# Prachet-Dev-Singh/DenseCLIP_Vit_multimodal

Measured on AMD Instinct MI355X. Metric: images/sec (fwd+bwd) ViT-B/16 DenseCLIP @1024x2048, higher is better.
Workload: dtype bf16

## Files before the change

denseclip_vit_multimodal_amd/_native.py:

```python
import ctypes
import os
import threading

_HERE = os.path.dirname(os.path.abspath(__file__))
LIB_PATH = os.environ.get("DCLIP_LIB", os.path.join(_HERE, "libdclip.so"))

F32, F16, BF16 = 0, 1, 2
EPI_STORE, EPI_GELU, EPI_RESIDUAL, EPI_GELU_BWD, EPI_SPLITK, EPI_STORE_SCALED = 0, 1, 2, 3, 4, 5
OPT_ATTN_FWD_WAVES, OPT_ATTN_DQ_WAVES, OPT_ATTN_DKDV_WAVES, OPT_GEMM_TILE, OPT_GEMM_TN_TILE = 0, 1, 2, 3, 4
OPT_ATTN_DKDV_QS, OPT_ATTN_FWD_KERNEL, OPT_ATTN_BWD_KERNEL, OPT_ATTN_BWD_BLOCK, OPT_GEMM_TN_COLSUM = 5, 6, 7, 8, 9
OPT_GEMM_EPI, OPT_GEMM_TAIL, OPT_ATTN_FP8_QK, OPT_ATTN_DQ_ISSUE, OPT_ATTN_DQ_ROWS = 10, 11, 12, 13, 14
OPT_ATTN_DQ_DEFER, OPT_GEMM_SCHED, OPT_GEMM_KLOOP = 15, 16, 17
OPT_ATTN_DQ_REDUCE = 18
OPT_ATTN_PREP_ORDER = 19
OPT_ATTN_BWD_WGS = 20
OPT_ATTN_DQ_DEFER = 15

_c_void_p = ctypes.c_void_p
_i32 = ctypes.c_int
_i64 = ctypes.c_int64
_f32 = ctypes.c_float

_SIGS = {
    "dclip_layernorm_fwd": [_c_void_p, _i32, _c_void_p, _c_void_p, _c_void_p, _i32, _c_void_p, _c_void_p,
                            _i64, _i64, _f32, _c_void_p],
    "dclip_layernorm_bwd": [_c_void_p, _i32, _c_void_p, _i32, _c_void_p, _c_void_p, _c_void_p, _c_void_p, _i32,
                            _c_void_p, _c_void_p, _i64, _i64, _c_void_p],
    "dclip_layernorm_bwd_res": [_c_void_p, _i32, _c_void_p, _i64, _c_void_p, _i32, _c_void_p, _c_void_p, _c_void_p,
                                _c_void_p, _c_void_p, _c_void_p, _i32, _c_void_p, _c_void_p, _c_void_p, _i64, _i64,
                                _c_void_p],
    "dclip_layernorm_bwd_ws_floats": [_i64, _i64],
    "dclip_layernorm_bwd_add": [_c_void_p, _i32, _c_void_p, _c_void_p, _c_void_p, _c_void_p, _c_void_p, _c_void_p,
                                _i32, _c_void_p, _c_void_p, _i32, _c_void_p, _c_void_p, _c_void_p, _i64, _i64,
                                _c_void_p],
    "dclip_layernorm_bwd_scaled_add": [_c_void_p, _i32, _c_void_p, _c_void_p, _c_void_p, _c_void_p, _c_void_p,
                                       _c_void_p, _c_void_p, _i32, _c_void_p, _i32, _c_void_p, _c_void_p, _c_void_p,
                                       _c_void_p, _c_void_p, _i64, _i64, _f32, _c_void_p, _i32, _c_void_p, _c_void_p],
    "dclip_gemm": [_i32, _i32, _c_void_p, _i64, _c_void_p, _i64, _i64, _i64, _i64, _i32, _f32, _c_void_p, _c_void_p,
                   _c_void_p,
                   _i32, _i64, _c_void_p, _i32, _i64, _c_void_p, _i64, _c_void_p],
    "dclip_gemm_tn": [_i32, _i32, _c_void_p, _i64, _c_void_p, _i64, _i64, _i64, _i64, _i64, _i32, _f32, _c_void_p,
                      _c_void_p,
                      _c_void_p, _c_void_p, _i64, _c_void_p, _c_void_p],
    "dclip_attn_fwd": [_i32, _c_void_p, _c_void_p, _c_void_p, _i32, _i32, _i32, _i32, _f32, _c_void_p],
    "dclip_attn_bwd": [_i32, _c_void_p, _c_void_p, _c_void_p, _c_void_p, _c_void_p, _c_void_p, _i32, _i32, _i32,
                       _i32, _f32, _c_void_p],
    "dclip_im2col": [_c_void_p, _i32, _c_void_p, _i32, _i64, _i32, _i32, _i32, _i32, _i32, _c_void_p],
    "dclip_tokens_fwd": [_c_void_p, _i32, _c_void_p, _c_void_p, _c_void_p, _i32, _i32, _i32, _c_void_p],
    "dclip_tokens_bwd": [_c_void_p, _c_void_p, _i32, _f32, _c_void_p, _c_void_p, _c_void_p, _i32, _i32, _i32,
                         _c_void_p],
    "dclip_pos_interp_fwd": [_c_void_p, _c_void_p, _i32, _i32, _i32, _i32, _c_void_p],
    "dclip_pos_interp_bwd": [_c_void_p, _c_void_p, _i32, _i32, _i32, _i32, _c_void_p],
    "dclip_transpose": [_c_void_p, _i32, _i64, _i64, _i64, _c_void_p, _i32, _i64, _i64, _i32, _i64, _i64, _i64,
                        _i32, _c_void_p, _c_void_p],
    "dclip_weight_refresh": [_c_void_p, _i32, _i64, _i32, _c_void_p],
    "dclip_row_mean_workspace": [_i32, _i64, _i32],
    "dclip_row_mean": [_c_void_p, _i32, _i64, _i64, _i64, _i32, _i64, _i32, _c_void_p, _c_void_p, _c_void_p],
    "dclip_score_map": [_c_void_p, _i32, _i64, _i64, _i64, _c_void_p, _c_void_p, _i32, _i32, _i32, _i32, _f32,
                        _c_void_p],
    "dclip_score_concat": [_c_void_p, _i32, _i64, _i64, _i64, _i32, _c_void_p, _i32, _i32, _i32, _c_void_p, _i32, _i32,
                           _i32, _c_void_p],
    "dclip_bilinear_fwd": [_c_void_p, _i32, _c_void_p, _i32, _i64, _i32, _i32, _i32, _i32, _c_void_p],
    "dclip_bilinear_bwd": [_c_void_p, _i32, _c_void_p, _c_void_p, _i64, _i32, _i32, _i32, _i32, _c_void_p],
    "dclip_cast": [_c_void_p, _i32, _c_void_p, _i32, _i64, _f32, _c_void_p, _c_void_p],
    "dclip_grad_scale": [_c_void_p, _i64, _f32, _c_void_p, _c_void_p],
    "dclip_cityscapes_augment": [_c_void_p, _c_void_p, _c_void_p, _i32, _i32, _i32, _c_void_p, _i32, _i32,
                                 _c_void_p, _c_void_p, _f32, _f32, _c_void_p, _i32, _c_void_p, _c_void_p, _c_void_p,
                                 _c_void_p],
    "dclip_color_jitter": [_c_void_p, _i32, _i32, _i32, _c_void_p, _c_void_p, _c_void_p],
    "dclip_normalize_u8": [_c_void_p, _i32, _i32, _i32, _c_void_p, _c_void_p, _c_void_p, _i32, _c_void_p],
    "dclip_bn_eval": [_i32, _c_void_p, _i64, _i32, _i64, _c_void_p, _c_void_p, _f32, _c_void_p, _c_void_p,
                      _c_void_p, _c_void_p, _i32, _c_void_p],
    "dclip_row_scale_add": [_c_void_p, _c_void_p, _c_void_p, _i32, _c_void_p, _i64, _i32, _c_void_p],
    "dclip_add_readout_amax": [_c_void_p, _c_void_p, _i32, _c_void_p, _c_void_p, _i64, _i32, _i32, _f32, _c_void_p,
                               _c_void_p],
    "dclip_add_readout_cast": [_c_void_p, _c_void_p, _i32, _c_void_p, _c_void_p, _i32, _i64, _i32, _i32, _f32,
                               _c_void_p],
    "dclip_add_readout_cast_scaled": [_c_void_p, _c_void_p, _i32, _c_void_p, _c_void_p, _c_void_p, _i64, _i32, _i32,
                                      _f32, _c_void_p, _i32, _c_void_p, _c_void_p],
    "dclip_layernorm_bwd_scaled": [_c_void_p, _i32, _c_void_p, _c_void_p, _i32, _c_void_p, _c_void_p, _c_void_p,
                                   _c_void_p, _c_void_p, _c_void_p, _c_void_p, _c_void_p, _c_void_p, _i64, _i64, _f32,
                                   _c_void_p, _i32, _c_void_p, _c_void_p],
    "dclip_bn_workspace": [_i64, _i32],
    "dclip_bn_fwd": [_i32, _c_void_p, _i64, _i32, _i64, _c_void_p, _c_void_p, _f32, _f32, _c_void_p, _c_void_p,
                     _c_void_p, _c_void_p, _c_void_p, _c_void_p, _i32, _c_void_p],
    "dclip_bn_bwd": [_i32, _c_void_p, _c_void_p, _i64, _i32, _i64, _c_void_p, _c_void_p, _c_void_p, _c_void_p,
                     _c_void_p, _c_void_p, _c_void_p, _c_void_p, _i32, _c_void_p, _c_void_p],
    "dclip_conv3x3": [_i32, _i32, _c_void_p, _i64, _i64, _i64, _i32, _i32, _i32, _i32, _c_void_p, _i32, _c_void_p,
                      _i32, _i64, _i32, _i32, _i32, _c_void_p],
    "dclip_upsample_ce": [_i32, _c_void_p, _i32, _i32, _i32, _i32, _c_void_p, _i32, _i32, _i32, _i32, _c_void_p,
                          _c_void_p, _c_void_p, _c_void_p, _c_void_p],
    "dclip_upsample_silog": [_i32, _i32, _c_void_p, _i32, _i32, _i32, _c_void_p, _c_void_p, _i32, _i32, _f32, _f32,
                             _c_void_p, _c_void_p, _c_void_p, _c_void_p],
    "dclip_upsample_ws_floats": [_i32, _i32, _i32, _i32],
    "dclip_upsample_eval_ws_bytes": [_i32, _i32, _i32, _i32],
    "dclip_upsample_eval_seg": [_i32, _c_void_p, _i32, _i32, _i32, _i32, _c_void_p, _i32, _i32, _i32, _i32,
                                _c_void_p, _c_void_p, _c_void_p, _c_void_p, _c_void_p, _c_void_p],
    "dclip_upsample_eval_depth": [_i32, _c_void_p, _i32, _i32, _i32, _c_void_p, _c_void_p, _i32, _i32, _f32, _f32,
                                  _i32, _f32, _c_void_p, _c_void_p, _c_void_p, _c_void_p],
    "dclip_score_map_classes": [_c_void_p, _i32, _i64, _i64, _i64, _c_void_p, _c_void_p, _i32, _i32, _i32, _i32,
                                _f32, _c_void_p],
    "dclip_upsample_ce_classes_ws_floats": [_i32, _i32, _i32, _i32],
    "dclip_upsample_ce_classes": [_i32, _c_void_p, _i32, _i32, _i32, _i32, _c_void_p, _i32, _i32, _i32, _i32,
                                  _c_void_p, _c_void_p, _c_void_p, _c_void_p, _c_void_p],
    "dclip_upsample_ce_opt_ws_floats": [_i32, _i32, _i32, _i32],
    "dclip_upsample_ce_opt": [_i32, _c_void_p, _i32, _i32, _i32, _i32, _c_void_p, _i32, _i32, _i32, _i32,
                              _c_void_p, _f32, _c_void_p, _c_void_p, _c_void_p, _c_void_p, _c_void_p, _c_void_p,
                              _c_void_p],
    "dclip_upsample_eval_seg_classes_ws_bytes": [_i32, _i32, _i32, _i32],
    "dclip_upsample_eval_seg_classes": [_i32, _c_void_p, _i32, _i32, _i32, _i32, _c_void_p, _i32, _i32, _i32, _i32,
                                        _c_void_p, _c_void_p, _c_void_p, _c_void_p, _c_void_p, _c_void_p],
    "dclip_ensemble_eval_ws_bytes": [_i32, _i32, _i32],
    "dclip_ensemble_eval_seg": [_i32, _c_void_p, _i32, _i32, _i32, _i32, _c_void_p, _i32, _i32, _i32, _i32,
                                _c_void_p, _c_void_p, _c_void_p, _c_void_p, _c_void_p, _c_void_p],
    "dclip_ensemble_eval_depth": [_i32, _c_void_p, _i32, _i32, _c_void_p, _c_void_p, _i32, _i32, _f32, _f32,
                                  _i32, _f32, _c_void_p, _c_void_p, _c_void_p, _c_void_p],
    "dclip_slide_eval_ws_bytes": [_i32, _i32, _i32],
    "dclip_slide_eval_seg": [_i32, _c_void_p, _i32, _i32, _i32, _i32, _i32, _i32, _i32, _c_void_p, _i32, _i32, _i32,
                             _i32, _c_void_p, _c_void_p, _c_void_p, _c_void_p, _c_void_p, _c_void_p],
    "dclip_slide_eval_depth": [_i32, _c_void_p, _i32, _i32, _i32, _i32, _i32, _i32, _c_void_p, _c_void_p, _i32, _i32,
                               _f32, _f32, _i32, _f32, _c_void_p, _c_void_p, _c_void_p, _c_void_p],
    "dclip_slide_tta_eval_ws_bytes": [_i32, _i32, _i32, _i32],
    "dclip_slide_tta_eval_seg": [_i32, _c_void_p, _i32, _c_void_p, _i32, _i32, _i32, _i32, _c_void_p, _i32, _i32,
                                 _i32, _i32, _c_void_p, _c_void_p, _c_void_p, _c_void_p, _c_void_p, _c_void_p],
    "dclip_slide_tta_eval_depth": [_i32, _c_void_p, _i32, _c_void_p, _i32, _i32, _c_void_p, _c_void_p, _i32, _i32,
                                   _f32, _f32, _i32, _f32, _c_void_p, _c_void_p, _c_void_p, _c_void_p],
    "dclip_conv3x3_wgrad": [_i32, _c_void_p, _i64, _i32, _c_void_p, _i64, _i64, _i64, _i32, _i32, _i32, _i32,
                            _c_void_p, _c_void_p, _i32, _i32, _c_void_p, _c_void_p],
    "dclip_set_option": [_i32, _i32],
    "dclip_cityscapes_prepare": [_c_void_p, _c_void_p, _c_void_p, _i32, _i32, _i32, _c_void_p, _i32, _i32,
                                 _c_void_p, _c_void_p, _f32, _f32, _c_void_p, _i32, _c_void_p, _c_void_p, _c_void_p,
                                 _c_void_p],
    "dclip_attn_bwd_workspace": [_i32, _i32, _i32],
    "dclip_attn_bwd_fp8_workspace": [_i32, _i32, _i32],
    "dclip_attn_bwd_fp8": [_i32, _c_void_p, _c_void_p, _c_void_p, _c_void_p, _c_void_p, _c_void_p, _i32, _i32, _i32,
                           _i32, _f32, _c_void_p],
    "dclip_attn_fwd_fp8": [_i32, _c_void_p, _c_void_p, _c_void_p, _c_void_p, _i32, _i32, _i32, _i32, _c_void_p],
    "dclip_attn_fwd_fp8_workspace": [_i32, _i32, _i32],
    "dclip_gemm_tn_plan": [_i64, _i64, _i64, _c_void_p, _c_void_p],
    "dclip_adamw_ws_bytes": [_i64],
    "dclip_adamw_prepare": [_c_void_p, _c_void_p, _c_void_p, _i32, _i64, _c_void_p, _i32, _c_void_p, _c_void_p,
                            _c_void_p, _i32, _c_void_p],
    "dclip_adamw_update": [_c_void_p, _c_void_p, _c_void_p, _i32, _i64, _c_void_p, _c_void_p],
}
EXPORTED = sorted(list(_SIGS) + ["dclip_last_error", "dclip_abi_version"])
ENSEMBLE_MAX_VIEWS = 16
CLASSES_MAX = 256


class View(ctypes.Structure):
    _fields_ = [("low", ctypes.c_void_p), ("h", ctypes.c_int), ("w", ctypes.c_int), ("flip", ctypes.c_int)]


def view_table(views):
    return (View * len(views))(*[View(p, int(h), int(w), int(f)) for p, h, w, f in views])


SLIDE_MAX_WINDOWS = 64


class Window(ctypes.Structure):
    _fields_ = [("low", ctypes.c_void_p), ("y0", ctypes.c_int), ("x0", ctypes.c_int)]


def window_table(windows):
    return (Window * len(windows))(*[Window(p, int(y), int(x)) for p, y, x in windows])


SLIDE_TTA_MAX_WINDOWS = 1024


class SlideView(ctypes.Structure):
    _fields_ = [(n, ctypes.c_int) for n in ("Hv", "Wv", "flip", "wh", "ww", "h", "w", "first", "nwin")]


def slide_view_table(views):
    return (SlideView * len(views))(*[SlideView(*[int(c) for c in v]) for v in views])


_lib = None
_lock = threading.Lock()


class NativeError(RuntimeError):
    pass


def load(path=None):
    global _lib
    with _lock:
        if _lib is not None and path is None:
            return _lib
        p = path or LIB_PATH
        if not os.path.exists(p):
            raise NativeError(
                f"libdclip.so not found at {p}: build it with `make -C denseclip_vit_multimodal_amd/csrc` "
                "(the HIP path has no CPU fallback)")
        lib = ctypes.CDLL(p)
        for name, args in _SIGS.items():
            fn = getattr(lib, name)
            fn.argtypes = args
            fn.restype = ctypes.c_int
        lib.dclip_last_error.restype = ctypes.c_char_p
        lib.dclip_last_error.argtypes = []
        lib.dclip_abi_version.restype = ctypes.c_int
        lib.dclip_abi_version.argtypes = []
        lib.dclip_attn_bwd_workspace.restype = ctypes.c_int64
        lib.dclip_attn_bwd_fp8_workspace.restype = ctypes.c_int64
        lib.dclip_bn_workspace.restype = ctypes.c_int64
        lib.dclip_attn_fwd_fp8_workspace.restype = ctypes.c_int64
        lib.dclip_row_mean_workspace.restype = ctypes.c_int64
        lib.dclip_layernorm_bwd_ws_floats.restype = ctypes.c_int64
        lib.dclip_upsample_ws_floats.restype = ctypes.c_int64
        lib.dclip_upsample_eval_ws_bytes.restype = ctypes.c_int64
        lib.dclip_upsample_ce_classes_ws_floats.restype = ctypes.c_int64
        lib.dclip_upsample_ce_opt_ws_floats.restype = ctypes.c_int64
        lib.dclip_upsample_eval_seg_classes_ws_bytes.restype = ctypes.c_int64
        lib.dclip_adamw_ws_bytes.restype = ctypes.c_int64
        lib.dclip_ensemble_eval_ws_bytes.restype = ctypes.c_int64
        lib.dclip_slide_eval_ws_bytes.restype = ctypes.c_int64
        lib.dclip_slide_tta_eval_ws_bytes.restype = ctypes.c_int64
        for kv in filter(None, os.environ.get("DCLIP_OPTIONS", "").split(",")):
            k, v = kv.split("=")
            if lib.dclip_set_option(int(k), int(v)) != 0:
                raise NativeError(f"DCLIP_OPTIONS: {lib.dclip_last_error().decode()}")
        if path is None:
            _lib = lib
        return lib


def lib():
    return load()


def call(name, *args):
    L = load()
    rc = getattr(L, name)(*args)
    if rc != 0:
        msg = L.dclip_last_error().decode(errors="replace")
        raise NativeError(f"{name} failed ({rc}): {msg}")
    return rc
```

denseclip_vit_multimodal_amd/_torch_ops.py:

```python
import os

import torch

_HERE = os.path.dirname(os.path.abspath(__file__))
LIB_PATH = os.environ.get("DCLIP_TORCH_LIB", os.path.join(_HERE, "libdclip_torch.so"))

_loaded = False


def load():
    global _loaded
    if _loaded:
        return torch.ops.dclip
    if not os.path.exists(LIB_PATH):
        raise RuntimeError(f"libdclip_torch.so not found at {LIB_PATH}: build it with "
                           "`make -C denseclip_vit_multimodal_amd/csrc` (the HIP path has no CPU fallback)")
    from . import _native
    bound = os.path.realpath(os.path.join(os.path.dirname(LIB_PATH), "libdclip.so"))
    if os.path.realpath(_native.LIB_PATH) != bound:
        raise RuntimeError(f"DCLIP_LIB ({_native.LIB_PATH}) is not the libdclip.so that {LIB_PATH} binds ({bound}); "
                           "build a matching adapter and point DCLIP_TORCH_LIB at it")
    _native.load()
    torch.ops.load_library(LIB_PATH)
    _register_fakes()
# ... 211 lines not shown
    @reg("dclip_eval::seg_update")
    def _(logits, labels, ignore_index, cm, ce_sums, want_pred):
        return _e(*labels.shape, like=logits, dtype=torch.uint8) if want_pred else None

    @reg("dclip_eval::depth_update")
    def _(pred, target, mask, min_depth, max_depth, clamp_pred, eps, sums, want_up):
        B, H, W = target.shape
        return _e(B, 1, H, W, like=pred, dtype=f32) if want_up else None

    @reg("dclip_eval::ensemble_argmax")
    def _(logits, flips, H, W, probs):
        return _e(logits[0].shape[0], H, W, like=logits[0], dtype=torch.uint8)

    @reg("dclip_eval::ensemble_seg_update")
    def _(logits, flips, labels, ignore_index, probs, cm, ce_sums, want_pred):
        return _e(*labels.shape, like=logits[0], dtype=torch.uint8) if want_pred else None

    @reg("dclip_eval::ensemble_depth")
    def _(preds, flips, H, W):
        return _e(preds[0].shape[0], 1, H, W, like=preds[0], dtype=f32)

    @reg("dclip_eval::ensemble_depth_update")
    def _(preds, flips, target, mask, min_depth, max_depth, clamp_pred, eps, sums, want_up):
        B, H, W = target.shape
        return _e(B, 1, H, W, like=preds[0], dtype=f32) if want_up else None

    @reg("dclip_eval::slide_argmax")
    def _(logits, origins, wh, ww, H, W):
        return _e(logits[0].shape[0], H, W, like=logits[0], dtype=torch.uint8)

    @reg("dclip_eval::slide_seg_update")
    def _(logits, origins, wh, ww, labels, ignore_index, cm, ce_sums, want_pred):
        return _e(*labels.shape, like=logits[0], dtype=torch.uint8) if want_pred else None

    @reg("dclip_eval::slide_depth")
    def _(preds, origins, wh, ww, H, W):
        return _e(preds[0].shape[0], 1, H, W, like=preds[0], dtype=f32)

    @reg("dclip_eval::slide_depth_update")
    def _(preds, origins, wh, ww, target, mask, min_depth, max_depth, clamp_pred, eps, sums, want_up):
        B, H, W = target.shape
        return _e(B, 1, H, W, like=preds[0], dtype=f32) if want_up else None

    @reg("dclip_eval::slide_tta_argmax")
    def _(logits, views, origins, H, W, probs):
        return _e(logits[0].shape[0], H, W, like=logits[0], dtype=torch.uint8)

    @reg("dclip_eval::slide_tta_seg_update")
    def _(logits, views, origins, labels, ignore_index, probs, cm, ce_sums, want_pred):
        return _e(*labels.shape, like=logits[0], dtype=torch.uint8) if want_pred else None

    @reg("dclip_eval::slide_tta_depth")
    def _(preds, views, origins, H, W):
        return _e(preds[0].shape[0], 1, H, W, like=preds[0], dtype=f32)

    @reg("dclip_eval::slide_tta_depth_update")
    def _(preds, views, origins, target, mask, min_depth, max_depth, clamp_pred, eps, sums, want_up):
        B, H, W = target.shape
        return _e(B, 1, H, W, like=preds[0], dtype=f32) if want_up else None

    @reg("dclip_eval::upsample_argmax_classes")
    def _(logits, H, W):
        return _e(logits.shape[0], H, W, like=logits, dtype=torch.uint8)

    @reg("dclip_eval::seg_update_classes")
    def _(logits, labels, ignore_index, cm, ce_sums, want_pred, ws=None):
        return _e(*labels.shape, like=logits, dtype=torch.uint8) if want_pred else None

    @reg("dclip_classes::score_map")
    def _(v, bstride, row_off, ld, text, B, HW, eps):
        return _e(B, text.shape[1], HW, like=v, dtype=f32)

    @reg("dclip_classes::upsample_ce")
    def _(logits, labels, ignore_index):
        return (_e(1, like=logits, dtype=torch.float64), _e(1, like=logits, dtype=torch.int32),
                _e(*logits.shape, like=logits, dtype=f32))

    @reg("dclip_loss::upsample_ce")
    def _(logits, labels, ignore_index, class_weight, label_smoothing, pixel_weight, want_pixel_loss, want_grad):
        return (_e(2, like=logits, dtype=torch.float64), _e(1, like=logits, dtype=torch.int32),
                _e(*logits.shape, like=logits, dtype=f32) if want_grad else None,
                _e(*labels.shape, like=logits, dtype=f32) if want_pixel_loss else None)

    @reg("dclip_optim::adamw_prepare")
    def _(desc, desc_host, grads, tiles, hp, found_inf, state, with_norm):
        return None

    @reg("dclip_optim::adamw_update")
    def _(desc, desc_host, grads, tiles, state):
        return None
```

denseclip_vit_multimodal_amd/csrc/gemm.hip:

```cpp
#include <mutex>
#include <type_traits>

#include "common.h"

namespace {

constexpr int BM = 128, BN = 128, BK = 64;
constexpr int TILE_BYTES = 128 * BK * 2;
constexpr int STAGE_BYTES = 2 * TILE_BYTES;
constexpr int EP_LD = 68;
constexpr int SMEM_BYTES = 4 * 64 * EP_LD * 4 > 2 * STAGE_BYTES ? 4 * 64 * EP_LD * 4 : 2 * STAGE_BYTES;

template <typename T>
__device__ __forceinline__ void store8(T* p, const float* v, bool full, int rem) {
    if (full) {
        if constexpr (sizeof(T) == 4) {
            f32x4 a = {v[0], v[1], v[2], v[3]}, b = {v[4], v[5], v[6], v[7]};
            *(f32x4*)p = a;
            *(f32x4*)(p + 4) = b;
        } else {
            typedef T t8 __attribute__((ext_vector_type(8)));
            t8 x;
#pragma unroll
            for (int e = 0; e < 8; ++e) x[e] = (T)v[e];
// ... 719 lines not shown
            for (int q = 0; q < 4; ++q) {
                const int rr = (lane >> 4) + 4 * q, cc = lane & 15;
                f32x4 x = *(const f32x4*)(img + rr * 256 + ((cc ^ (rr & 15)) * 16));
                const int64_t row = row0 + rr;
                const int col = nw + 4 * cc;
                if constexpr (EPI == DCLIP_EPI_RESIDUAL) {
                    x += cur[q];
                    st16<NTS>((f32x4*)((float*)C + row * ldc + col), x);
                    if (C2 != nullptr) {
                        const t4 y = {(T)x[0], (T)x[1], (T)x[2], (T)x[3]};
                        *(t4*)((T*)C2 + row * ldc2 + col) = y;
                    }
                } else if constexpr (EPI == DCLIP_EPI_GELU_BWD) {
#pragma unroll
                    for (int e = 0; e < 4; ++e) x[e] *= quick_gelu_grad((float)cur[q][e]);
                    store4_out<OutT>((OutT*)C + row * ldc + col, x);
                } else {
                    store4_out<OutT>((OutT*)C + row * ldc + col, x);
                }
            }
        } else {
#pragma unroll
            for (int q = 0; q < 2; ++q) {
                const int rr = (lane >> 3) + 8 * q, cc = lane & 7;
                const int off = rr * 128 + ((cc ^ ((rr >> 1) & 7)) * 16);
                const int64_t row = row0 + rr;
                const int col = nw + 8 * cc;
                if (EPI != DCLIP_EPI_GELU || C != nullptr)
                    st16<NTS>((u32x4*)((OutT*)C + row * ldc + col), *(const u32x4*)(img + off));
                if constexpr (EPI == DCLIP_EPI_GELU)
                    st16<NTS>((u32x4*)((OutT*)C2 + row * ldc2 + col), *(const u32x4*)(img + 2048 + off));
            }
        }
        asm volatile("" ::: "memory");
        if constexpr (AUX) {
            if (j + 1 < Cfg::MB) {
#pragma unroll
                for (int q = 0; q < 4; ++q) cur[q] = nxt[q];
            }
        }
    }
}

__device__ __forceinline__ void pers_range(int x, int G, int ntiles, int& lo, int& hi) {
    const int rest = ntiles - G;
    lo = G + (int)((int64_t)rest * x / 8);
    hi = G + (int)((int64_t)rest * (x + 1) / 8);
}

__device__ __forceinline__ int pers_resolve(unsigned* __restrict__ sched, int v, int xcd, int G, int ntiles) {
    int lo, hi;
    pers_range(xcd, G, ntiles, lo, hi);
    if (lo + v < hi) return lo + v;
#pragma unroll 1
    for (int k = 1; k < 8; ++k) {
        const int x = (xcd + k) & 7;
        pers_range(x, G, ntiles, lo, hi);
        if (lo >= hi) continue;
        const int w = (int)atomicAdd(sched + 32 * x, 1u);
        if (lo + w < hi) return lo + w;
    }
    unsigned* const bm = sched + 288;
#pragma unroll 1
    for (int w = 0; w < (G + 31) / 32; ++w) {
        const unsigned valid = (w * 32 + 32 <= G) ? 0xffffffffu : ((1u << (G - w * 32)) - 1u);
        unsigned bits = atomicOr(bm + w, 0u);
        while ((~bits & valid) != 0u) {
            const int bit = __builtin_ctz(~bits & valid);
            const unsigned old = atomicOr(bm + w, 1u << bit);
            if (!(old & (1u << bit))) return w * 32 + bit;
            bits |= old;
        }
    }
    if ((int)atomicAdd(sched + 256, 1u) == G - 1) {
#pragma unroll 1
        for (int i = 0; i < 8; ++i) atomicExch(sched + 32 * i, 0u);
        atomicExch(sched + 256, 0u);
#pragma unroll 1
        for (int i = 288; i < 296; ++i) atomicExch(sched + i, 0u);
    }
    return ntiles;
}

template <typename T, int EPI, typename OutT, int NW = 8, bool ELDS = false, bool DYN = false, bool NTS = false,
          bool PF = false>
__global__ __launch_bounds__(64 * NW, 1) void gemm_nt_pers_kernel(
    const T* __restrict__ A, int64_t lda, const T* __restrict__ B, int64_t ldb, int K, int tiles_m, int tiles_n,
    const float* __restrict__ bias, const void* __restrict__ aux, int64_t ld_aux, void* __restrict__ C, int64_t ldc,
    void* __restrict__ C2, int64_t ldc2, Alpha alpha_arg, unsigned* __restrict__ sched = nullptr) {
    const float alpha = alpha_arg.get();
    typedef BigCfg<256, 256, 2, NW / 2, 2, 64> Cfg;
    typedef typename Mfma<T>::frag frag;
    constexpr int EPI_IMG = (NW == 8 && ELDS) ? 4096 : 0;
    __shared__ __attribute__((aligned(16))) char smem[Cfg::SMEM + NW * EPI_IMG];
    const int lane = threadIdx.x & 63;
    const int wave = __builtin_amdgcn_readfirstlane(threadIdx.x >> 6);
    const int wm = wave / (NW / 2), wn = wave % (NW / 2);
    constexpr bool epi_lds = NW == 8 && ELDS;
    const int l16 = lane & 15, lq = lane >> 4;
    const int ntiles = tiles_m * tiles_n;
    const int G = gridDim.x;
    const int r = xcd_remap(blockIdx.x, G);
    const int nk = K / 64;
    const int M = tiles_m * 256, N = tiles_n * 256;

    const uint32_t abytes = (uint32_t)((int64_t)M * lda * sizeof(T)), bbytes = (uint32_t)((int64_t)N * ldb * sizeof(T));
    const uint32_t lda_b = (uint32_t)(lda * sizeof(T)), ldb_b = (uint32_t)(ldb * sizeof(T));
    uint32_t va[2], vb[2];
    rows_voff2<Cfg::A_INST>(lda_b, lane, va);
    rows_voff2<Cfg::B_INST>(ldb_b, lane, vb);
#define PERS_STAGE(M0, N0, KT, SLOT)                                                                                 \
    do {                                                                                                             \
        char* base_ = smem + (SLOT) * Cfg::STAGE_BYTES;                                                              \
        const uint32_t kb_ = (uint32_t)((KT) * 64 * sizeof(T));                                                      \
        stage_rows_sbuf<T, Cfg::A_INST>(A, abytes, va, (uint32_t)((M0) + 8 * wave * Cfg::A_INST) * lda_b + kb_,     \
                                        8 * lda_b, base_, wave);                                                     \
        stage_rows_sbuf<T, Cfg::B_INST>(B, bbytes, vb, (uint32_t)((N0) + 8 * wave * Cfg::B_INST) * ldb_b + kb_,     \
                                        8 * ldb_b, base_ + Cfg::A_BYTES, wave);                                      \
    } while (0)
    int u = r;
    if (u >= ntiles) return;
    int m0 = (u / tiles_n) * 256, n0 = (u % tiles_n) * 256;
    int* const pub = (int*)(smem + Cfg::SMEM);
    const int xcd = blockIdx.x & 7;
    unsigned own_old = 0;
    int pend = 0;
    if constexpr (DYN) {
        static_assert(!DYN || (NW == 8 && ELDS), "the claim words live in wave 0's epilogue image");
        if (threadIdx.x == 0) {
            own_old = atomicOr(sched + 288 + (r >> 5), 1u << (r & 31));
            pend = (int)atomicAdd(sched + 32 * xcd, 1u);
        }
    }
    PERS_STAGE(m0, n0, 0, 0);
    int slot = 0;
    bool first = true;
    while (true) {
        f32x4 acc[Cfg::NB][Cfg::MB];
#pragma unroll
        for (int i = 0; i < Cfg::NB; ++i)
#pragma unroll
            for (int j = 0; j < Cfg::MB; ++j) acc[i][j] = f32x4{0.f, 0.f, 0.f, 0.f};
        PersCols<EPI, Cfg::NB> pc;
        pers_cols<EPI, Cfg::NB>(pc, bias, aux, n0 + wn * Cfg::WTN, lq);
        int un = u + G;
        if constexpr (DYN) {
            if (nk == 2 && threadIdx.x == 0) {
                pub[0] = pers_resolve(sched, pend, xcd, G, ntiles);
                asm volatile("s_waitcnt lgkmcnt(0)" ::: "memory");
            }
        }
        int nm0 = (un / tiles_n) * 256, nn0 = (un % tiles_n) * 256;
        bool skip = false;
        for (int kt = 0; kt < nk; ++kt) {
            if (kt == 0 && !first) wait_vmcnt<PERS_EPI_MIN>();
            else wait_vmcnt<0>();
            if constexpr (DYN) {
                if (kt == 0 && first && u == r && threadIdx.x == 0) {
                    pub[1] = (own_old >> (r & 31)) & 1u;
                    asm volatile("s_waitcnt lgkmcnt(0)" ::: "memory");
                }
            }
            __builtin_amdgcn_s_barrier();
            __builtin_amdgcn_sched_barrier(0);
            if constexpr (DYN) {
                if (kt == 0 && first && u == r && __builtin_amdgcn_readfirstlane(pub[1]) != 0) {
                    skip = true;
                    break;
                }
                if (kt == nk - 2) {
                    un = __builtin_amdgcn_readfirstlane(pub[0]);
                    nm0 = (un / tiles_n) * 256;
                    nn0 = (un % tiles_n) * 256;
                }
            }
            if (kt + 1 < nk) {
                PERS_STAGE(m0, n0, kt + 1, slot ^ 1);
            } else if (un < ntiles) {
                PERS_STAGE(nm0, nn0, 0, slot ^ 1);
            }
            const char* At = smem + slot * Cfg::STAGE_BYTES;
            const char* Bt = At + Cfg::A_BYTES;
            if constexpr (PF && NW == 8) {
                frag fb[2][Cfg::NB], fa[4];
                auto rd_b = [&](int ks) {
#pragma unroll
                    for (int i = 0; i < Cfg::NB; ++i)
// ... 885 lines not shown
            __syncthreads();
        }
    }
    if constexpr (AD) __syncthreads();
    gemm_epilogue<T, DCLIP_EPI_SPLITK, float>(acc, smem, M, N, m0, n0, nullptr, nullptr, 0, C, N, nullptr, 0, slab,
                                               1.0f);
}

const void* conv_zero_row() {
    static void* z = nullptr;
    if (!z) {
        if (hipMalloc(&z, 256) != hipSuccess) return nullptr;
        if (hipMemset(z, 0, 256) != hipSuccess) return nullptr;
    }
    return z;
}

float* tail_scratch(size_t floats) {
    static float* buf = nullptr;
    static size_t cap = 0;
    if (floats > cap) {
        if (buf) (void)hipFree(buf);
        buf = nullptr;
        cap = 0;
        if (hipMalloc(&buf, floats * sizeof(float)) != hipSuccess) return nullptr;
        cap = floats;
    }
    return buf;
}

template <typename T, int EPI, typename OutT>
__global__ __launch_bounds__(512) void gemm_tail16_kernel(const T* __restrict__ A, int64_t lda, const T* __restrict__ B,
                                                          int64_t ldb, int mt, int N, int K, int m0,
                                                          const float* __restrict__ bias, const void* __restrict__ aux,
                                                          int64_t ld_aux, void* __restrict__ C, int64_t ldc,
                                                          void* __restrict__ C2, int64_t ldc2, Alpha alpha_arg) {
    typedef typename Mfma<T>::frag frag;
    __shared__ float red[8][16][68];
    const int lane = threadIdx.x & 63, wave = threadIdx.x >> 6;
    const int l16 = lane & 15, lq = lane >> 4;
    const int n0 = blockIdx.x * 64;
    const int ks = K / 8, kbeg = wave * ks;
    const bool rowok = l16 < mt;
    const T* arow = A + (int64_t)(rowok ? l16 : 0) * lda + kbeg + 8 * lq;
    const T* brow = B + (int64_t)(n0 + l16) * ldb + kbeg + 8 * lq;
    f32x4 acc[4];
#pragma unroll
    for (int i = 0; i < 4; ++i) acc[i] = f32x4{0.f, 0.f, 0.f, 0.f};
    frag zf;
#pragma unroll
    for (int j = 0; j < 8; ++j) zf[j] = (T)0.f;
#pragma unroll 4
    for (int k = 0; k < ks; k += 32) {
        const frag a = rowok ? *(const frag*)(arow + k) : zf;
        frag b[4];
#pragma unroll
        for (int i = 0; i < 4; ++i) b[i] = *(const frag*)(brow + (int64_t)16 * i * ldb + k);
#pragma unroll
        for (int i = 0; i < 4; ++i) acc[i] = Mfma16<T>::mma(a, b[i], acc[i]);
    }
#pragma unroll
    for (int i = 0; i < 4; ++i)
#pragma unroll
        for (int e = 0; e < 4; ++e) red[wave][4 * lq + e][16 * i + l16] = acc[i][e];
    __syncthreads();
    const int t = threadIdx.x;
    if (t < 128) {
        const int r = t >> 3, cb = (t & 7) * 8;
        if (r < mt) {
            const float alpha = alpha_arg.get();
            float v[8];
#pragma unroll
            for (int e = 0; e < 8; ++e) {
                float sum = 0.f;
#pragma unroll
                for (int w = 0; w < 8; ++w) sum += red[w][r][cb + e];
                v[e] = sum * alpha;
            }
            epi_row8<T, EPI, OutT>(v, m0 + r, n0 + cb, N, bias, aux, ld_aux, C, ldc, C2, ldc2, 0);
        }
    }
}

template <typename T, int EPI, typename OutT>
__global__ __launch_bounds__(1024) void gemm_tail16x16_kernel(const T* __restrict__ A, int64_t lda,
                                                              const T* __restrict__ B, int64_t ldb, int mt, int N,
                                                              int W, int IT, int m0, const float* __restrict__ bias,
                                                              const void* __restrict__ aux, int64_t ld_aux,
                                                              void* __restrict__ C, int64_t ldc, void* __restrict__ C2,
                                                              int64_t ldc2, Alpha alpha_arg) {
    typedef typename Mfma<T>::frag frag;
    constexpr int ITMAX = 6;
    __shared__ float red[16][16][17];
    const int lane = threadIdx.x & 63, wave = threadIdx.x >> 6;
    const int l16 = lane & 15, lq = lane >> 4;
    const int n0 = blockIdx.x * 16;
    const int t = threadIdx.x;
    const int er = t >> 1, ecb = (t & 1) * 8;
    const bool epi = t < 2 * mt;
    float bv[8], pre[8];
#pragma unroll
    for (int e = 0; e < 8; ++e) bv[e] = pre[e] = 0.f;
    if (epi) {
        const int nb = n0 + ecb;
        if (bias != nullptr && EPI != DCLIP_EPI_GELU_BWD) load8<float>(bias + nb, bv, true, 8);
        if constexpr (EPI == DCLIP_EPI_STORE_SCALED) load8<float>((const float*)aux + nb, pre, true, 8);
        if constexpr (EPI == DCLIP_EPI_RESIDUAL)
            load8<float>((const float*)aux + (int64_t)(m0 + er) * ld_aux + nb, pre, true, 8);
        if constexpr (EPI == DCLIP_EPI_GELU_BWD) load8<T>((const T*)aux + (int64_t)(m0 + er) * ld_aux + nb, pre, true, 8);
    }
    const bool rowok = l16 < mt;
    const int kbeg = wave * IT * 32;
    const T* arow = A + (int64_t)(rowok ? l16 : 0) * lda + kbeg + 8 * lq;
    const T* brow = B + (int64_t)(n0 + l16) * ldb + kbeg + 8 * lq;
    frag zf;
#pragma unroll
    for (int j = 0; j < 8; ++j) zf[j] = (T)0.f;
    frag a[ITMAX], b[ITMAX];
#pragma unroll
    for (int it = 0; it < ITMAX; ++it) {
        if (it < IT) {
            a[it] = rowok ? *(const frag*)(arow + 32 * it) : zf;
            b[it] = *(const frag*)(brow + 32 * it);
        }
    }
    f32x4 acc = f32x4{0.f, 0.f, 0.f, 0.f};
#pragma unroll
    for (int it = 0; it < ITMAX; ++it)
        if (it < IT) acc = Mfma16<T>::mma(a[it], b[it], acc);
#pragma unroll
    for (int e = 0; e < 4; ++e) red[wave][4 * lq + e][l16] = acc[e];
    __syncthreads();
    if (epi) {
        const float alpha = alpha_arg.get();
        float v[8];
#pragma unroll
        for (int e = 0; e < 8; ++e) {
            float sum = 0.f;
            for (int w = 0; w < W; ++w) sum += red[w][er][ecb + e];
            v[e] = sum * alpha + bv[e];
        }
        const int64_t m = m0 + er;
        const int nb = n0 + ecb;
        if constexpr (EPI == DCLIP_EPI_STORE) {
            store8<OutT>((OutT*)C + m * ldc + nb, v, true, 8);
        } else if constexpr (EPI == DCLIP_EPI_STORE_SCALED) {
#pragma unroll
            for (int e = 0; e < 8; ++e) v[e] *= pre[e];
            store8<OutT>((OutT*)C + m * ldc + nb, v, true, 8);
        } else if constexpr (EPI == DCLIP_EPI_GELU) {
            float g[8];
#pragma unroll
            for (int e = 0; e < 8; ++e) {
                v[e] = (float)(OutT)v[e];
                g[e] = quick_gelu(v[e]);
            }
            if (C != nullptr) store8<OutT>((OutT*)C + m * ldc + nb, v, true, 8);
            store8<OutT>((OutT*)C2 + m * ldc2 + nb, g, true, 8);
        } else if constexpr (EPI == DCLIP_EPI_RESIDUAL) {
#pragma unroll
            for (int e = 0; e < 8; ++e) v[e] += pre[e];
            store8<float>((float*)C + m * ldc + nb, v, true, 8);
            if (C2 != nullptr) store8<T>((T*)C2 + m * ldc2 + nb, v, true, 8);
        } else if constexpr (EPI == DCLIP_EPI_GELU_BWD) {
#pragma unroll
            for (int e = 0; e < 8; ++e) v[e] *= quick_gelu_grad(pre[e]);
            store8<OutT>((OutT*)C + m * ldc + nb, v, true, 8);
        }
    }
}

inline bool tail16x16_plan(int64_t K, int& W, int& IT) {
    if (K % 32 != 0) return false;
    const int s = (int)(K / 32);
    for (int w = 16; w >= 1; --w)
        if (s % w == 0 && s / w <= 6) {
            W = w;
            IT = s / w;
            return true;
        }
    return false;
}

template <typename T, int EPI, typename OutT>
__global__ void tail_combine_kernel(const float* __restrict__ ws, int splits, int rows, int N, int64_t m0,
                                    const float* __restrict__ bias, const void* __restrict__ aux, int64_t ld_aux,
                                    void* __restrict__ C, int64_t ldc, void* __restrict__ C2, int64_t ldc2) {
    const int n8 = (N + 7) / 8;
    const int i = blockIdx.x * blockDim.x + threadIdx.x;
    if (i >= rows * n8) return;
    const int r = i / n8, nb = (i % n8) * 8;
    const bool full = nb + 8 <= N;
    float v[8] = {0.f, 0.f, 0.f, 0.f, 0.f, 0.f, 0.f, 0.f};
    for (int sp = 0; sp < splits; ++sp) {
        float t[8];
        load8<float>(ws + ((int64_t)sp * rows + r) * N + nb, t, full, N - nb);
#pragma unroll
        for (int e = 0; e < 8; ++e) v[e] += t[e];
    }
    epi_row8<T, EPI, OutT>(v, (int)(m0 + r), nb, N, bias, aux, ld_aux, C, ldc, C2, ldc2, 0);
}

template <typename T, int EPI, typename OutT, int TBM, int TBN, int WM, int WN, int STAGES, int BKT = 64,
          bool PP = false>
void launch_big(const void* A, int64_t lda, const void* B, int64_t ldb, int64_t M, int64_t N, int64_t K,
                int splits, Alpha alpha, const float* bias, const void* aux, int64_t ld_aux, void* C, int64_t ldc,
                void* C2, int64_t ldc2, hipStream_t st) {
    int tiles_m = (int)((M + TBM - 1) / TBM);
    const int tiles_n = (int)((N + TBN - 1) / TBN);
    const int64_t Mfull = (M / TBM) * TBM, tail = M - Mfull;
    auto rounds = [](int64_t t) { return (t + 255) / 256; };
    if (EPI != DCLIP_EPI_SPLITK && splits == 1 && tail > 0 && tail <= 64 && Mfull > 0 && K >= 1536 &&
        rounds((int64_t)tiles_m * tiles_n) > rounds((Mfull / TBM) * tiles_n)) {
        const int ksteps = (int)(K / BKT);
        int ts = 1;
        for (int c = 16; c >= 1; --c)
            if (ksteps % c == 0) {
                ts = c;
                break;
            }
        float* ws = tail_scratch((size_t)ts * tail * N);
        if (ws != nullptr) {
            tiles_m = (int)(Mfull / TBM);
            const int ttm = 1;
            gemm_nt_big_kernel<T, DCLIP_EPI_SPLITK, float, TBM, TBN, WM, WN, STAGES, BKT>
                <<<dim3(ttm * tiles_n, ts), 64 * WM * WN, 0, st>>>(
                    (const T*)A + Mfull * lda, lda, (const T*)B, ldb, (int)tail, (int)N, (int)(K / ts), ttm, tiles_n,
                    nullptr, nullptr, 0, ws, N, nullptr, 0, tail * N, alpha);
            const int threads = (int)(tail * ((N + 7) / 8));
            tail_combine_kernel<T, EPI, OutT><<<(threads + 255) / 256, 256, 0, st>>>(
                ws, ts, (int)tail, (int)N, Mfull, bias, aux, ld_aux, C, ldc, C2, ldc2);
            M = Mfull;
        }
    }
    dim3 grid(tiles_m * tiles_n, splits);
    if constexpr (PP) {
        static_assert(TBM == 256 && TBN == 256 && WM == 2 && WN == 4, "ping-pong geometry");
        gemm_nt_pp_kernel<T, EPI, OutT><<<grid, 512, 0, st>>>(
            (const T*)A, lda, (const T*)B, ldb, (int)M, (int)N, (int)(K / splits), tiles_m, tiles_n, bias, aux, ld_aux,
            C, ldc, C2, ldc2, (int64_t)M * N, alpha);
    } else {
        gemm_nt_big_kernel<T, EPI, OutT, TBM, TBN, WM, WN, STAGES, BKT><<<grid, 64 * WM * WN, 0, st>>>(
            (const T*)A, lda, (const T*)B, ldb, (int)M, (int)N, (int)(K / splits), tiles_m, tiles_n, bias, aux,
            ld_aux, C, ldc, C2, ldc2, (int64_t)M * N, alpha);
    }
}

int cu_count() {
    static int n[64] = {0};
    int dev = 0;
    (void)hipGetDevice(&dev);
    if (dev < 0 || dev >= 64) return 256;
    if (n[dev] == 0) {
        int c = 0;
        if (hipDeviceGetAttribute(&c, hipDeviceAttributeMultiprocessorCount, dev) != hipSuccess || c <= 0) c = 256;
        n[dev] = c;
    }
    return n[dev];
}

unsigned* gemm_sched_counters(hipStream_t st) {
    static std::mutex mu;
    static unsigned* base[64] = {nullptr};
    static hipStream_t owner[64][64];
    static int used[64] = {0};
    if (dclip_option(DCLIP_OPT_GEMM_SCHED) != 1) return nullptr;
    hipStreamCaptureStatus cs = hipStreamCaptureStatusNone;
    if (hipStreamIsCapturing(st, &cs) != hipSuccess || cs != hipStreamCaptureStatusNone) return nullptr;
    int dev = 0;
    if (hipGetDevice(&dev) != hipSuccess || dev < 0 || dev >= 64) return nullptr;
    std::lock_guard<std::mutex> lock(mu);
    if (base[dev] == nullptr) {
        unsigned* p = nullptr;
        const size_t bytes = 64 * 512 * sizeof(unsigned);
        if (hipMalloc(&p, bytes) != hipSuccess) return nullptr;
        if (hipMemset(p, 0, bytes) != hipSuccess) {
            (void)hipFree(p);
            return nullptr;
        }
        base[dev] = p;
    }
    for (int i = 0; i < used[dev]; ++i)
        if (owner[dev][i] == st) return base[dev] + 512 * i;
    if (used[dev] == 64) return nullptr;
    owner[dev][used[dev]] = st;
    return base[dev] + 512 * used[dev]++;
}

inline bool pers_streaming_stores(int epi, int64_t N) {
    const int o = dclip_option(DCLIP_OPT_GEMM_EPI);
    if (o == 2) return true;
    if (o != 0) return false;
    return N >= 2048 && epi != DCLIP_EPI_GELU_BWD && epi != DCLIP_EPI_RESIDUAL;
}

inline bool pers_prefetch_kloop(int epi) {
    const int o = dclip_option(DCLIP_OPT_GEMM_KLOOP);
    if (o == 1) return true;
    if (o != 0) return false;
    return epi != DCLIP_EPI_GELU;
}

template <typename T, int EPI, typename OutT, int NW = 8, bool PIPE = false>
bool launch_pers(const void* A, int64_t lda, const void* B, int64_t ldb, int64_t M, int64_t N, int64_t K,
                 Alpha alpha, const float* bias, const void* aux, int64_t ld_aux, void* C, int64_t ldc, void* C2,
                 int64_t ldc2, hipStream_t st) {
    if constexpr (EPI == DCLIP_EPI_SPLITK) {
        return false;
    } else {
        const int64_t Mfull = (M / 256) * 256, tail = M - Mfull;
        const int G = cu_count();
        if (N % 256 != 0 || tail > 64 || (Mfull / 256) * (N / 256) < 2 * G) return false;
        if (PIPE && K < 128) return false;
        if (Mfull * lda * (int64_t)sizeof(T) >= (1ll << 32) || N * ldb * (int64_t)sizeof(T) >= (1ll << 32)) return false;
        if (EPI == DCLIP_EPI_STORE_SCALED || (bias != nullptr && EPI != DCLIP_EPI_GELU_BWD)) {
            if (((uintptr_t)(EPI == DCLIP_EPI_STORE_SCALED ? aux : bias) % 16) != 0) return false;
            if (bias != nullptr && ((uintptr_t)bias % 16) != 0) return false;
        }
        if (ldc % 4 != 0 || (C2 != nullptr && ldc2 % 4 != 0) || (EPI == DCLIP_EPI_RESIDUAL && ld_aux % 4 != 0) ||
            (EPI == DCLIP_EPI_GELU_BWD && ld_aux % 4 != 0))
            return false;
        const int tail_opt = dclip_option(DCLIP_OPT_GEMM_TAIL);
        int tw = 0, tit = 0;
        if (tail > 0 && tail <= 16 && tail_opt == 0 && tail16x16_plan(K, tw, tit)) {
            gemm_tail16x16_kernel<T, EPI, OutT><<<(unsigned)(N / 16), 64 * tw, 0, st>>>(
                (const T*)A + Mfull * lda, lda, (const T*)B, ldb, (int)tail, (int)N, tw, tit, (int)Mfull, bias, aux,
                ld_aux, C, ldc, C2, ldc2, alpha);
        } else if (tail > 0 && tail <= 16 && K % 256 == 0 && tail_opt != 1) {
            gemm_tail16_kernel<T, EPI, OutT><<<(unsigned)(N / 64), 512, 0, st>>>(
                (const T*)A + Mfull * lda, lda, (const T*)B, ldb, (int)tail, (int)N, (int)K, (int)Mfull, bias, aux,
                ld_aux, C, ldc, C2, ldc2, alpha);
        } else if (tail > 0) {
            const int tiles_n = (int)(N / 256);
            const int ksteps = (int)(K / 64);
            int ts = 1;
            for (int c = 16; c >= 1; --c)
                if (ksteps % c == 0) {
                    ts = c;
                    break;
                }
            float* ws = tail_scratch((size_t)ts * tail * N);
            if (ws == nullptr) return false;
            gemm_nt_big_kernel<T, DCLIP_EPI_SPLITK, float, 256, 256, 2, 4, 2, 64>
                <<<dim3(tiles_n, ts), 512, 0, st>>>((const T*)A + Mfull * lda, lda, (const T*)B, ldb, (int)tail, (int)N,
                                                    (int)(K / ts), 1, tiles_n, nullptr, nullptr, 0, ws, N, nullptr, 0,
                                                    tail * N, alpha);
            const int threads = (int)(tail * ((N + 7) / 8));
            tail_combine_kernel<T, EPI, OutT><<<(threads + 255) / 256, 256, 0, st>>>(
                ws, ts, (int)tail, (int)N, Mfull, bias, aux, ld_aux, C, ldc, C2, ldc2);
        }
        if constexpr (PIPE)
            gemm_nt_pipe_kernel<T, EPI, OutT, NW><<<G, 64 * NW, 0, st>>>((const T*)A, lda, (const T*)B, ldb, (int)K,
                                                                         (int)(Mfull / 256), (int)(N / 256), bias, aux,
                                                                         ld_aux, C, ldc, C2, ldc2, alpha);
        else
        {
            unsigned* sched = (NW == 8 && dclip_option(DCLIP_OPT_GEMM_EPI) != 1 && K >= 128 && G <= 256)
                                  ? gemm_sched_counters(st)
                                  : nullptr;
            if (sched != nullptr)
                gemm_nt_pers_kernel<T, EPI, OutT, NW, true, NW == 8><<<G, 64 * NW, 0, st>>>(
                    (const T*)A, lda, (const T*)B, ldb, (int)K, (int)(Mfull / 256), (int)(N / 256), bias, aux, ld_aux, C,
                    ldc, C2, ldc2, alpha, sched);
#define PERS_LAUNCH(NTS_, PF_)                                                                                  \
    gemm_nt_pers_kernel<T, EPI, OutT, NW, true, false, NTS_, PF_><<<G, 64 * NW, 0, st>>>(                        \
        (const T*)A, lda, (const T*)B, ldb, (int)K, (int)(Mfull / 256), (int)(N / 256), bias, aux, ld_aux, C, ldc, C2, \
        ldc2, alpha)
            else if (NW == 8 && dclip_option(DCLIP_OPT_GEMM_EPI) != 1) {
                const bool nts = pers_streaming_stores(EPI, N), pf = pers_prefetch_kloop(EPI);
                if (nts && pf) PERS_LAUNCH(true, true);
                else if (nts) PERS_LAUNCH(true, false);
                else if (pf) PERS_LAUNCH(false, true);
                else PERS_LAUNCH(false, false);
            }
#undef PERS_LAUNCH
            else
                gemm_nt_pers_kernel<T, EPI, OutT, NW, false><<<G, 64 * NW, 0, st>>>(
                    (const T*)A, lda, (const T*)B, ldb, (int)K, (int)(Mfull / 256), (int)(N / 256), bias, aux, ld_aux, C,
                    ldc, C2, ldc2, alpha);
        }
        return true;
    }
}

inline int gemm_tile_choice(int64_t M, int64_t N) {
    const int opt = dclip_option(DCLIP_OPT_GEMM_TILE);
    if (opt != 0) return opt;
    if (M < 4096) return 1;
    return 6;
}

template <typename T, int EPI, typename OutT>
int launch(const void* A, int64_t lda, const void* B, int64_t ldb, int64_t M, int64_t N, int64_t K,
           int splits, Alpha alpha, const float* bias, const void* aux, int64_t ld_aux, void* C, int64_t ldc,
           void* C2, int64_t ldc2, hipStream_t st) {
    const int choice = gemm_tile_choice(M, N);
    if (choice == 2) {
        launch_big<T, EPI, OutT, 256, 256, 2, 4, 2>(A, lda, B, ldb, M, N, K, splits, alpha, bias, aux, ld_aux, C,
                                                    ldc, C2, ldc2, st);
        return 0;
    }
    if (choice == 3) {
        launch_big<T, EPI, OutT, 256, 128, 4, 2, 3>(A, lda, B, ldb, M, N, K, splits, alpha, bias, aux, ld_aux, C,
                                                    ldc, C2, ldc2, st);
        return 0;
    }
    if (choice == 6 && splits == 1 &&
        launch_pers<T, EPI, OutT>(A, lda, B, ldb, M, N, K, alpha, bias, aux, ld_aux, C, ldc, C2, ldc2, st))
        return 0;
    if (choice == 7 && splits == 1 &&
        launch_pers<T, EPI, OutT, 4>(A, lda, B, ldb, M, N, K, alpha, bias, aux, ld_aux, C, ldc, C2, ldc2, st))
        return 0;
    if (choice == 8 && splits == 1 &&
        launch_pers<T, EPI, OutT, 8, true>(A, lda, B, ldb, M, N, K, alpha, bias, aux, ld_aux, C, ldc, C2, ldc2, st))
        return 0;
    if (choice == 9 && splits == 1 &&
        launch_pers<T, EPI, OutT, 4, true>(A, lda, B, ldb, M, N, K, alpha, bias, aux, ld_aux, C, ldc, C2, ldc2, st))
        return 0;
    if (choice >= 6) {
        launch_big<T, EPI, OutT, 256, 256, 2, 4, 2>(A, lda, B, ldb, M, N, K, splits, alpha, bias, aux, ld_aux, C,
                                                    ldc, C2, ldc2, st);
        return 0;
    }
    if (choice == 5) {
        launch_big<T, EPI, OutT, 256, 256, 2, 4, 2, 64, true>(A, lda, B, ldb, M, N, K, splits, alpha, bias, aux,
                                                              ld_aux, C, ldc, C2, ldc2, st);
        return 0;
    }
    if (choice == 4) {
        launch_big<T, EPI, OutT, 256, 256, 2, 4, 4, 32>(A, lda, B, ldb, M, N, K, splits, alpha, bias, aux, ld_aux, C,
                                                        ldc, C2, ldc2, st);
        return 0;
    }
    const int tiles_m = (int)((M + BM - 1) / BM), tiles_n = (int)((N + BN - 1) / BN);
    const int k_chunk = (int)(K / splits);
    dim3 grid(tiles_m * tiles_n, splits);
    gemm_nt_kernel<T, EPI, OutT><<<grid, 256, 0, st>>>(
        (const T*)A, lda, (const T*)B, ldb, (int)M, (int)N, k_chunk, tiles_m, tiles_n, bias, aux,
        ld_aux, C, ldc, C2, ldc2, (int64_t)M * N, alpha);
    return 0;
}

template <typename T>
int dispatch(int epi, int c_dt, const void* A, int64_t lda, const void* B, int64_t ldb, int64_t M,
             int64_t N, int64_t K, int splits, Alpha alpha, const float* bias, const void* aux, int64_t ld_aux,
             void* C, int64_t ldc, void* C2, int64_t ldc2, hipStream_t st) {
    switch (epi) {
        case DCLIP_EPI_STORE:
            if (c_dt == DCLIP_F32)
                return launch<T, DCLIP_EPI_STORE, float>(A, lda, B, ldb, M, N, K, 1, alpha, bias, aux, ld_aux, C, ldc, C2, ldc2, st);
            return launch<T, DCLIP_EPI_STORE, T>(A, lda, B, ldb, M, N, K, 1, alpha, bias, aux, ld_aux, C, ldc, C2, ldc2, st);
        case DCLIP_EPI_STORE_SCALED:
            return launch<T, DCLIP_EPI_STORE_SCALED, T>(A, lda, B, ldb, M, N, K, 1, alpha, bias, aux, ld_aux, C, ldc, C2, ldc2, st);
        case DCLIP_EPI_GELU:
            return launch<T, DCLIP_EPI_GELU, T>(A, lda, B, ldb, M, N, K, 1, alpha, bias, aux, ld_aux, C, ldc, C2, ldc2, st);
        case DCLIP_EPI_RESIDUAL:
            return launch<T, DCLIP_EPI_RESIDUAL, float>(A, lda, B, ldb, M, N, K, 1, alpha, bias, aux, ld_aux, C, ldc, C2, ldc2, st);
        case DCLIP_EPI_GELU_BWD:
            return launch<T, DCLIP_EPI_GELU_BWD, T>(A, lda, B, ldb, M, N, K, 1, alpha, bias, aux, ld_aux, C, ldc, C2, ldc2, st);
        case DCLIP_EPI_SPLITK: {
            float* ws = (float*)const_cast<void*>(aux);
            launch<T, DCLIP_EPI_SPLITK, float>(A, lda, B, ldb, M, N, K, splits, alpha, nullptr, nullptr, 0,
// ... 275 lines not shown
```

denseclip_vit_multimodal_amd/csrc/misc.hip:

```cpp
#include "common.h"

namespace {

template <typename T>
__device__ __forceinline__ T cvt(float v) { return (T)v; }

template <typename TI, typename TO>
__global__ void im2col_kernel(const TI* __restrict__ img, TO* __restrict__ out, int B, int Cin, int Hin, int Win,
                              int p, int gh, int gw, int64_t ldo, int64_t total4) {
    const int64_t i = (int64_t)blockIdx.x * blockDim.x + threadIdx.x;
    if (i >= total4) return;
    const int64_t l4 = ldo / 4;
    const int64_t row = i / l4;
    const int col = (int)(i % l4) * 4;
    TO* dst = out + row * ldo + col;
    if (col >= Cin * p * p) {
#pragma unroll
        for (int e = 0; e < 4; ++e) dst[e] = (TO)0.0f;
        return;
    }
    const int kx = col % p, ky = (col / p) % p, cc = col / (p * p);
    const int px = (int)(row % gw);
    const int py = (int)((row / gw) % gh);
    const int b = (int)(row / ((int64_t)gw * gh));
// ... 894 lines not shown
    }
}

template <typename TB>
__global__ __launch_bounds__(256) void add_readout_cast_ds_kernel(const float* a, const TB* __restrict__ b,
                                                                  const float* __restrict__ bsc, float* sum,
                                                                  f16* __restrict__ lp, int64_t rows, int cols,
                                                                  int ntok, float target, float* __restrict__ st,
                                                                  int use, float* __restrict__ spair) {
    const int c8 = cols / 8;
    const int64_t n8 = rows * c8;
    const float sb = bsc != nullptr ? *bsc : 1.0f;
    const float ls = ds_scale_of_use(st, use, target);
    ds_begin(st, use, ls, spair);
    uint32_t m = 0;
    const int64_t stride = (int64_t)gridDim.x * blockDim.x;
    for (int64_t i = (int64_t)blockIdx.x * blockDim.x + threadIdx.x; i < n8; i += 2 * stride) {
        const int64_t i2 = i + stride;
        const bool two = i2 < n8;
        f32x4 x[4];
        readout_sum8<TB>(a, b, sb, i * 8, (i / c8) % ntok != 0, x[0], x[1]);
        if (two) readout_sum8<TB>(a, b, sb, i2 * 8, (i2 / c8) % ntok != 0, x[2], x[3]);
#pragma unroll
        for (int h = 0; h < 2; ++h) {
            if (h == 1 && !two) break;
            const int64_t off = (h ? i2 : i) * 8;
            if (b != nullptr) {
                *(f32x4*)(sum + off) = x[2 * h];
                *(f32x4*)(sum + off + 4) = x[2 * h + 1];
            }
            f16x8 o;
#pragma unroll
            for (int e = 0; e < 4; ++e) {
                m = max(m, max(__float_as_uint(x[2 * h][e]) & 0x7fffffffu, __float_as_uint(x[2 * h + 1][e]) & 0x7fffffffu));
                o[e] = (f16)(x[2 * h][e] * ls);
                o[4 + e] = (f16)(x[2 * h + 1][e] * ls);
            }
            *(f16x8*)(lp + off) = o;
        }
    }
    ds_end<4>(m, st, use);
}

extern "C" int dclip_add_readout_cast_scaled(const float* a, const void* b, int b_dt, const float* b_scale_ptr,
                                             float* sum, void* lp, int64_t rows, int cols, int ntok, float target,
                                             float* st, int use, float* spair, void* stream) {
    DCLIP_HOST_CHECK(cols % 8 == 0 && ntok > 0 && rows > 0 && target > 0.f && st != nullptr && spair != nullptr &&
                         use >= 1,
                     "dclip_add_readout_cast_scaled: cols %% 8 == 0, ntok > 0, rows > 0, target > 0, st, use >= 1, spair");
    DCLIP_HOST_CHECK(b == nullptr || sum != nullptr, "dclip_add_readout_cast_scaled: sum is required with b");
    DCLIP_HOST_CHECK(((uintptr_t)a | (uintptr_t)b | (uintptr_t)sum | (uintptr_t)lp) % 16 == 0,
                     "dclip_add_readout_cast_scaled: unaligned buffers");
    hipStream_t s = (hipStream_t)stream;
    const unsigned g = grid_for((rows * (cols / 8) + 1) / 2, 4096);
    if (b == nullptr) b_dt = DCLIP_F32;
    DISPATCH_DT(b_dt, TB,
        add_readout_cast_ds_kernel<TB><<<g, 256, 0, s>>>(a, (const TB*)b, b_scale_ptr, sum, (f16*)lp, rows, cols, ntok,
                                                         target, st, use, spair));
    DCLIP_LAUNCH_CHECK();
    return 0;
}

extern "C" int dclip_cast(const void* in, int in_dt, void* out, int out_dt, int64_t n, float scale_v,
                          const float* scale_ptr, void* stream) {
    if (n == 0) return 0;
    const Alpha scale(scale_v, scale_ptr);
    hipStream_t st = (hipStream_t)stream;
    DISPATCH_DT(in_dt, TI, DISPATCH_DT(out_dt, TO,
        cast_kernel<TI, TO><<<grid_for((n + 3) / 4), 256, 0, st>>>((const TI*)in, (TO*)out, n, scale)));
    DCLIP_LAUNCH_CHECK();
    return 0;
}

namespace {

constexpr int BN_NBLK_MAX = 512;

inline int bn_nblk(int64_t rows, int C) {
    const int rpb = 256 / (C / 8);
    const int64_t need = (rows + rpb - 1) / rpb;
    return (int)(need < BN_NBLK_MAX ? need : BN_NBLK_MAX);
}

template <typename T>
__device__ __forceinline__ void load8(const T* p, float* v) {
    typedef T t8 __attribute__((ext_vector_type(8)));
    const t8 r = *(const t8*)p;
#pragma unroll
    for (int e = 0; e < 8; ++e) v[e] = (float)r[e];
}

__device__ __forceinline__ void bn_affine8(const float* w, const float* b, const float* mean, const float* rstd, int c0,
                                           float* sc, float* sh) {
#pragma unroll
    for (int e = 0; e < 8; ++e) {
        sc[e] = (w ? w[c0 + e] : 1.f) * rstd[c0 + e];
        sh[e] = (b ? b[c0 + e] : 0.f) - mean[c0 + e] * sc[e];
    }
}

template <typename T, int MODE, bool RELU>
__global__ void __launch_bounds__(256) bn_stats_kernel(const T* __restrict__ a, const T* __restrict__ x,
                                                       const float* __restrict__ w, const float* __restrict__ b,
                                                       const float* __restrict__ mean, const float* __restrict__ rstd,
                                                       int64_t rows, int C, int64_t ld, float* __restrict__ part) {
    __shared__ float red[2 * 2048];
    const int tpr = C / 8, rpb = 256 / tpr;
    const int c8 = threadIdx.x % tpr, rr = threadIdx.x / tpr;
    float s[8], q[8], ref[8], sc[8], sh[8];
#pragma unroll
    for (int e = 0; e < 8; ++e) s[e] = q[e] = 0.f;
    if (rr < rpb) {
        if (MODE == 0) load8(a + c8 * 8, ref);
        else
#pragma unroll
            for (int e = 0; e < 8; ++e) ref[e] = mean[c8 * 8 + e];
        if (RELU) bn_affine8(w, b, mean, rstd, c8 * 8, sc, sh);
#pragma unroll 4
        for (int64_t r = (int64_t)blockIdx.x * rpb + rr; r < rows; r += (int64_t)gridDim.x * rpb) {
            float v[8];
            load8(a + r * ld + c8 * 8, v);
            if (MODE == 0) {
#pragma unroll
                for (int e = 0; e < 8; ++e) {
                    const float d = v[e] - ref[e];
                    s[e] += d;
                    q[e] += d * d;
                }
            } else {
                float xv[8];
                load8(x + r * ld + c8 * 8, xv);
#pragma unroll
                for (int e = 0; e < 8; ++e) {
                    const float g = (!RELU || xv[e] * sc[e] + sh[e] > 0.f) ? v[e] : 0.f;
                    s[e] += g;
                    q[e] += g * (xv[e] - ref[e]);
                }
            }
        }
#pragma unroll
        for (int e = 0; e < 8; ++e) {
            red[rr * C + c8 * 8 + e] = s[e];
            red[2048 + rr * C + c8 * 8 + e] = q[e];
        }
    }
    __syncthreads();
    for (int c = threadIdx.x; c < C; c += 256) {
        float ss = 0.f, qq = 0.f;
        for (int k = 0; k < rpb; ++k) {
            ss += red[k * C + c];
            qq += red[2048 + k * C + c];
        }
        part[(int64_t)blockIdx.x * 2 * C + c] = ss;
        part[(int64_t)blockIdx.x * 2 * C + C + c] = qq;
    }
}

__device__ __forceinline__ void bn_reduce_parts(const float* __restrict__ part, int nblk, int C, int& c, float& S,
                                                float& Q) {
    __shared__ float red[2][32][8];
    const int lc = threadIdx.x & 7, grp = threadIdx.x >> 3;
    c = blockIdx.x * 8 + lc;
    float s = 0.f, q = 0.f;
    if (c < C) {
#pragma unroll 4
        for (int k = grp; k < nblk; k += 32) {
            s += part[(int64_t)k * 2 * C + c];
            q += part[(int64_t)k * 2 * C + C + c];
        }
    }
    red[0][grp][lc] = s;
    red[1][grp][lc] = q;
    __syncthreads();
    S = Q = 0.f;
    if (threadIdx.x < 8)
        for (int g = 0; g < 32; ++g) {
            S += red[0][g][lc];
            Q += red[1][g][lc];
        }
}

template <typename T>
__global__ void bn_fwd_finalize_kernel(const float* __restrict__ part, int nblk, const T* __restrict__ x, int64_t rows,
                                       int C, const float* __restrict__ w, const float* __restrict__ b, float eps,
                                       float momentum, float* __restrict__ rmean, float* __restrict__ rvar,
                                       float* __restrict__ mean, float* __restrict__ rstd, float* __restrict__ ss) {
    int c;
    float S, Q;
    bn_reduce_parts(part, nblk, C, c, S, Q);
    if (threadIdx.x >= 8 || c >= C) return;
    const float n = (float)rows;
    const float md = S / n;
    const float var = fmaxf(Q / n - md * md, 0.f);
    const float mu = (float)x[c] + md;
    const float rs = rsqrtf(var + eps);
    mean[c] = mu;
    rstd[c] = rs;
    const float sc = (w ? w[c] : 1.f) * rs;
    ss[c] = sc;
    ss[C + c] = (b ? b[c] : 0.f) - mu * sc;
    if (rmean) {
        rmean[c] = (1.f - momentum) * rmean[c] + momentum * mu;
        rvar[c] = (1.f - momentum) * rvar[c] + momentum * var * (rows > 1 ? n / (n - 1.f) : 1.f);
    }
}

__global__ void bn_bwd_finalize_kernel(const float* __restrict__ part, int nblk, int64_t rows, int C,
                                       const float* __restrict__ w, const float* __restrict__ mean,
                                       const float* __restrict__ rstd, float* __restrict__ dw, float* __restrict__ db,
                                       float* __restrict__ k, const float* __restrict__ gscale) {
    int c;
    float S, Q;
    bn_reduce_parts(part, nblk, C, c, S, Q);
    if (threadIdx.x >= 8 || c >= C) return;
    const float n = (float)rows, rs = rstd[c], wc = w ? w[c] : 1.f;
    const float ga = gscale ? *gscale : 1.f;
    if (dw) dw[c] = Q * rs * ga;
    if (db) db[c] = S * ga;
    const float k1 = wc * rs;
    const float k2 = -wc * rs * rs * rs * (Q / n);
    k[c] = k1;
    k[C + c] = k2;
    k[2 * C + c] = -k1 * (S / n) - k2 * mean[c];
}

template <typename T, bool BWD, bool RELU>
__global__ void __launch_bounds__(256) bn_apply_kernel(const T* __restrict__ a, const T* __restrict__ x,
                                                       const float* __restrict__ k, int64_t rows, int C, int64_t ld,
                                                       T* __restrict__ y) {
    const int c8n = C / 8;
    const int64_t n8 = rows * c8n;
    typedef T t8 __attribute__((ext_vector_type(8)));
    for (int64_t i = (int64_t)blockIdx.x * blockDim.x + threadIdx.x; i < n8; i += (int64_t)gridDim.x * blockDim.x) {
        const int c0 = (int)(i % c8n) * 8;
        const int64_t off = (i / c8n) * ld + c0;
        float v[8];
        load8(a + off, v);
        t8 o;
        if (BWD) {
            float xv[8];
            load8(x + off, xv);
#pragma unroll
            for (int e = 0; e < 8; ++e) {
                const float g = (!RELU || xv[e] * k[3 * C + c0 + e] + k[4 * C + c0 + e] > 0.f) ? v[e] : 0.f;
                o[e] = (T)(g * k[c0 + e] + xv[e] * k[C + c0 + e] + k[2 * C + c0 + e]);
            }
        } else {
#pragma unroll
            for (int e = 0; e < 8; ++e) {
                const float t = v[e] * k[c0 + e] + k[C + c0 + e];
                o[e] = (T)(RELU ? fmaxf(t, 0.f) : t);
            }
        }
        *(t8*)(y + off) = o;
    }
}

__global__ void bn_mask_affine_kernel(const float* __restrict__ w, const float* __restrict__ b,
                                      const float* __restrict__ mean, const float* __restrict__ rstd, int C,
                                      float* __restrict__ k) {
    const int c = blockIdx.x * 256 + threadIdx.x;
    if (c >= C) return;
    const float sc = (w ? w[c] : 1.f) * rstd[c];
    k[3 * C + c] = sc;
    k[4 * C + c] = (b ? b[c] : 0.f) - mean[c] * sc;
}

__global__ void bn_eval_affine_kernel(const float* __restrict__ w, const float* __restrict__ b,
                                      const float* __restrict__ rmean, const float* __restrict__ rvar, float eps,
                                      int C, float* __restrict__ ss) {
    const int c = blockIdx.x * 256 + threadIdx.x;
    if (c >= C) return;
    const float sc = (w ? w[c] : 1.f) / sqrtf(rvar[c] + eps);
    ss[c] = sc;
    ss[C + c] = (b ? b[c] : 0.f) - rmean[c] * sc;
}

bool bn_shape_ok(int64_t rows, int C, int64_t ld) {
    const int tpr = C / 8;
    return rows > 0 && C % 8 == 0 && tpr >= 1 && tpr <= 256 && ld >= C && ld % 8 == 0;
}

}

extern "C" int64_t dclip_bn_workspace(int64_t rows, int C) {
    (void)rows;
    return (int64_t)BN_NBLK_MAX * 2 * C + 5 * (int64_t)C;
}

extern "C" int dclip_bn_fwd(int dt, const void* x, int64_t rows, int C, int64_t ld, const float* w, const float* b,
                            float eps, float momentum, float* running_mean, float* running_var, float* ws, float* mean,
                            float* rstd, void* y, int relu, void* stream) {
    DCLIP_HOST_CHECK(dt == DCLIP_BF16 || dt == DCLIP_F16, "dclip_bn_fwd: dtype must be bf16/f16");
    DCLIP_HOST_CHECK(bn_shape_ok(rows, C, ld), "dclip_bn_fwd: need rows > 0, C %% 8 == 0, C <= 2048, ld >= C, "
                     "ld %% 8 == 0 (C = %d)", C);
    DCLIP_HOST_CHECK(((uintptr_t)x % 16) == 0 && ((uintptr_t)y % 16) == 0, "dclip_bn_fwd: unaligned buffers");
    hipStream_t st = (hipStream_t)stream;
    const int nblk = bn_nblk(rows, C);
    float* ss = ws + (int64_t)BN_NBLK_MAX * 2 * C;
    const unsigned ga = grid_for(rows * (C / 8), 8192);
#define BN_FWD(T)                                                                                                      \
    bn_stats_kernel<T, 0, false><<<nblk, 256, 0, st>>>((const T*)x, nullptr, nullptr, nullptr, nullptr, nullptr, rows, \
                                                       C, ld, ws);                                                     \
    bn_fwd_finalize_kernel<T><<<(C + 7) / 8, 256, 0, st>>>(ws, nblk, (const T*)x, rows, C, w, b, eps, momentum,        \
                                                           running_mean, running_var, mean, rstd, ss);                 \
    if (relu) bn_apply_kernel<T, false, true><<<ga, 256, 0, st>>>((const T*)x, nullptr, ss, rows, C, ld, (T*)y);       \
    else bn_apply_kernel<T, false, false><<<ga, 256, 0, st>>>((const T*)x, nullptr, ss, rows, C, ld, (T*)y);
    if (dt == DCLIP_BF16) {
        BN_FWD(bf16)
    } else {
        BN_FWD(f16)
    }
#undef BN_FWD
    DCLIP_LAUNCH_CHECK();
    return 0;
}

extern "C" int dclip_bn_eval(int dt, const void* x, int64_t rows, int C, int64_t ld, const float* w, const float* b,
                             float eps, const float* running_mean, const float* running_var, float* ws, void* y,
                             int relu, void* stream) {
    DCLIP_HOST_CHECK(dt == DCLIP_BF16 || dt == DCLIP_F16, "dclip_bn_eval: dtype must be bf16/f16");
    DCLIP_HOST_CHECK(bn_shape_ok(rows, C, ld), "dclip_bn_eval: need rows > 0, C %% 8 == 0, C <= 2048, ld >= C, "
                     "ld %% 8 == 0 (C = %d)", C);
    DCLIP_HOST_CHECK(running_mean && running_var && ws, "dclip_bn_eval: running statistics and workspace required");
    DCLIP_HOST_CHECK(((uintptr_t)x % 16) == 0 && ((uintptr_t)y % 16) == 0, "dclip_bn_eval: unaligned buffers");
    hipStream_t st = (hipStream_t)stream;
    float* ss = ws + (int64_t)BN_NBLK_MAX * 2 * C;
    const unsigned ga = grid_for(rows * (C / 8), 8192);
    bn_eval_affine_kernel<<<(C + 255) / 256, 256, 0, st>>>(w, b, running_mean, running_var, eps, C, ss);
#define BN_EVAL(T)                                                                                                 \
    if (relu) bn_apply_kernel<T, false, true><<<ga, 256, 0, st>>>((const T*)x, nullptr, ss, rows, C, ld, (T*)y);   \
    else bn_apply_kernel<T, false, false><<<ga, 256, 0, st>>>((const T*)x, nullptr, ss, rows, C, ld, (T*)y);
    if (dt == DCLIP_BF16) {
        BN_EVAL(bf16)
    } else {
        BN_EVAL(f16)
    }
#undef BN_EVAL
    DCLIP_LAUNCH_CHECK();
    return 0;
}

extern "C" int dclip_bn_bwd(int dt, const void* dy, const void* x, int64_t rows, int C, int64_t ld, const float* w,
                            const float* b, const float* mean, const float* rstd, float* ws, void* dx, float* dw,
                            float* db, int relu, const float* gscale, void* stream) {
    DCLIP_HOST_CHECK(dt == DCLIP_BF16 || dt == DCLIP_F16, "dclip_bn_bwd: dtype must be bf16/f16");
    DCLIP_HOST_CHECK(bn_shape_ok(rows, C, ld), "dclip_bn_bwd: need rows > 0, C %% 8 == 0, C <= 2048, ld >= C, "
                     "ld %% 8 == 0 (C = %d)", C);
    DCLIP_HOST_CHECK(((uintptr_t)dy % 16) == 0 && ((uintptr_t)x % 16) == 0 && ((uintptr_t)dx % 16) == 0,
                     "dclip_bn_bwd: unaligned buffers");
    hipStream_t st = (hipStream_t)stream;
    const int nblk = bn_nblk(rows, C);
    float* k = ws + (int64_t)BN_NBLK_MAX * 2 * C;
    const unsigned ga = grid_for(rows * (C / 8), 8192);
    if (relu) bn_mask_affine_kernel<<<(C + 255) / 256, 256, 0, st>>>(w, b, mean, rstd, C, k);
#define BN_BWD(T)                                                                                                      \
    if (relu) {                                                                                                        \
        bn_stats_kernel<T, 1, true><<<nblk, 256, 0, st>>>((const T*)dy, (const T*)x, w, b, mean, rstd, rows, C, ld, ws); \
        bn_bwd_finalize_kernel<<<(C + 7) / 8, 256, 0, st>>>(ws, nblk, rows, C, w, mean, rstd, dw, db, k, gscale);               \
        bn_apply_kernel<T, true, true><<<ga, 256, 0, st>>>((const T*)dy, (const T*)x, k, rows, C, ld, (T*)dx);          \
    } else {                                                                                                           \
        bn_stats_kernel<T, 1, false><<<nblk, 256, 0, st>>>((const T*)dy, (const T*)x, w, b, mean, rstd, rows, C, ld,   \
                                                           ws);                                                        \
        bn_bwd_finalize_kernel<<<(C + 7) / 8, 256, 0, st>>>(ws, nblk, rows, C, w, mean, rstd, dw, db, k, gscale);               \
        bn_apply_kernel<T, true, false><<<ga, 256, 0, st>>>((const T*)dy, (const T*)x, k, rows, C, ld, (T*)dx);         \
    }
    if (dt == DCLIP_BF16) {
        BN_BWD(bf16)
    } else {
        BN_BWD(f16)
    }
#undef BN_BWD
    DCLIP_LAUNCH_CHECK();
    return 0;
}
```

denseclip_vit_multimodal_amd/csrc/torch_ops.cpp:

```cpp
#include <ATen/ATen.h>
#include <c10/core/DeviceGuard.h>
#include <c10/hip/HIPStream.h>
#include <torch/library.h>

#include "../../include/dclip.h"

namespace {

using at::Tensor;

int dt_code(at::ScalarType t) {
    switch (t) {
        case at::kFloat: return DCLIP_F32;
        case at::kHalf: return DCLIP_F16;
        case at::kBFloat16: return DCLIP_BF16;
        default: TORCH_CHECK(false, "dclip: unsupported dtype ", t);
    }
    return -1;
}

void* stream_of(const Tensor& t) { return (void*)c10::hip::getCurrentHIPStream(t.device().index()).stream(); }

void check_gpu(const Tensor& t, const char* what, bool contiguous = true) {
    TORCH_CHECK(t.defined(), "dclip: ", what, " is undefined");
// ... 593 lines not shown

std::tuple<Tensor, Tensor> bn_fwd_into(const Tensor& x, const c10::optional<Tensor>& w, const c10::optional<Tensor>& b,
                                       const c10::optional<Tensor>& running_mean, const c10::optional<Tensor>& running_var,
                                       double momentum, double eps, bool relu, const Tensor& y) {
    const Rows r = rows_of(x), ry = rows_of(y);
    TORCH_CHECK(r.rows == ry.rows && r.C == ry.C && r.ld == ry.ld && x.scalar_type() == y.scalar_type(),
                "dclip: BatchNorm output must match the input's rows, channels and pitch");
    check_vec(w, r.C, "BatchNorm weight"); check_vec(b, r.C, "BatchNorm bias");
    check_vec(running_mean, r.C, "running_mean"); check_vec(running_var, r.C, "running_var");
    c10::DeviceGuard g(x.device());
    Tensor ws = at::empty({dclip_bn_workspace(r.rows, (int)r.C)}, like(x, at::kFloat));
    Tensor mean = at::empty({r.C}, like(x, at::kFloat)), rstd = at::empty({r.C}, like(x, at::kFloat));
    DCLIP_CALL(dclip_bn_fwd(dt_code(x.scalar_type()), x.data_ptr(), r.rows, (int)r.C, r.ld, optr<float>(w), optr<float>(b),
                            (float)eps, (float)momentum, optr<float>(running_mean), optr<float>(running_var),
                            ptr<float>(ws), ptr<float>(mean), ptr<float>(rstd), y.data_ptr(), relu ? 1 : 0, stream_of(x)));
    return {mean, rstd};
}

std::tuple<Tensor, Tensor, Tensor> bn_fwd(const Tensor& x, const c10::optional<Tensor>& w,
                                          const c10::optional<Tensor>& b, const c10::optional<Tensor>& running_mean,
                                          const c10::optional<Tensor>& running_var, double momentum, double eps,
                                          bool relu) {
    TORCH_CHECK(x.dim() == 4, "bn_fwd: a channels-last 4-D map");
    Tensor y = at::empty_like(x, at::MemoryFormat::ChannelsLast);
    auto ms = bn_fwd_into(x, w, b, running_mean, running_var, momentum, eps, relu, y);
    return {y, std::get<0>(ms), std::get<1>(ms)};
}

Tensor bn_eval(const Tensor& x, const c10::optional<Tensor>& w, const c10::optional<Tensor>& b,
               const Tensor& running_mean, const Tensor& running_var, double eps, bool relu) {
    TORCH_CHECK(x.dim() == 4, "bn_eval: a channels-last 4-D map");
    const Rows r = rows_of(x);
    check_vec(w, r.C, "BatchNorm weight"); check_vec(b, r.C, "BatchNorm bias");
    check_vec(running_mean, r.C, "running_mean"); check_vec(running_var, r.C, "running_var");
    c10::DeviceGuard g(x.device());
    Tensor y = at::empty_like(x, at::MemoryFormat::ChannelsLast);
    Tensor ws = at::empty({dclip_bn_workspace(r.rows, (int)r.C)}, like(x, at::kFloat));
    DCLIP_CALL(dclip_bn_eval(dt_code(x.scalar_type()), x.data_ptr(), r.rows, (int)r.C, r.ld, optr<float>(w),
                             optr<float>(b), (float)eps, ptr<float>(running_mean), ptr<float>(running_var),
                             ptr<float>(ws), y.data_ptr(), relu ? 1 : 0, stream_of(x)));
    return y;
}

std::tuple<Tensor, Tensor> bn_fwd_rows(const Tensor& x, const c10::optional<Tensor>& w, const c10::optional<Tensor>& b,
                                       c10::optional<Tensor> running_mean, c10::optional<Tensor> running_var,
                                       double momentum, double eps, bool relu, Tensor& y) {
    return bn_fwd_into(x, w, b, running_mean, running_var, momentum, eps, relu, y);
}

std::tuple<Tensor, Tensor> bn_bwd_into(const Tensor& dy, const Tensor& x, const c10::optional<Tensor>& w,
                                       const c10::optional<Tensor>& b, const Tensor& mean, const Tensor& rstd, bool relu,
                                       bool want_w, bool want_b, const Tensor& dx,
                                       const c10::optional<Tensor>& scale = c10::nullopt) {
    const Rows r = rows_of(x), rd = rows_of(dy), rdx = rows_of(dx);
    TORCH_CHECK(rd.rows == r.rows && rd.C == r.C && rd.ld == r.ld && rdx.ld == r.ld && rdx.rows == r.rows,
                "dclip: BatchNorm backward tensors must share rows, channels and pitch");
    TORCH_CHECK(dy.scalar_type() == x.scalar_type() && dx.scalar_type() == x.scalar_type(), "bn_bwd: dtypes must match");
    check_vec(w, r.C, "BatchNorm weight"); check_vec(b, r.C, "BatchNorm bias");
    check_vec(mean, r.C, "mean"); check_vec(rstd, r.C, "rstd");
    c10::DeviceGuard g(x.device());
    Tensor ws = at::empty({dclip_bn_workspace(r.rows, (int)r.C)}, like(x, at::kFloat));
    Tensor dw = want_w ? at::empty({r.C}, like(x, at::kFloat)) : at::empty({0}, like(x, at::kFloat));
    Tensor db = want_b ? at::empty({r.C}, like(x, at::kFloat)) : at::empty({0}, like(x, at::kFloat));
    DCLIP_CALL(dclip_bn_bwd(dt_code(x.scalar_type()), dy.data_ptr(), x.data_ptr(), r.rows, (int)r.C, r.ld, optr<float>(w),
                            optr<float>(b), ptr<float>(mean), ptr<float>(rstd), ptr<float>(ws), dx.data_ptr(),
                            want_w ? ptr<float>(dw) : nullptr, want_b ? ptr<float>(db) : nullptr, relu ? 1 : 0,
                            scale_entry(scale, 1), stream_of(x)));
    return {dw, db};
}

std::tuple<Tensor, Tensor, Tensor> bn_bwd(const Tensor& dy, const Tensor& x, const c10::optional<Tensor>& w,
                                          const c10::optional<Tensor>& b, const Tensor& mean, const Tensor& rstd,
                                          bool relu, bool want_w, bool want_b, const c10::optional<Tensor>& scale) {
    TORCH_CHECK(x.dim() == 4, "bn_bwd: a channels-last 4-D map");
    Tensor dx = at::empty_like(x, at::MemoryFormat::ChannelsLast);
    auto g = bn_bwd_into(dy, x, w, b, mean, rstd, relu, want_w, want_b, dx, scale);
    return {dx, std::get<0>(g), std::get<1>(g)};
}

std::tuple<Tensor, Tensor> bn_bwd_rows(const Tensor& dy, const Tensor& x, const c10::optional<Tensor>& w,
                                       const c10::optional<Tensor>& b, const Tensor& mean, const Tensor& rstd, bool relu,
                                       bool want_w, bool want_b, Tensor& dx, const c10::optional<Tensor>& scale) {
    return bn_bwd_into(dy, x, w, b, mean, rstd, relu, want_w, want_b, dx, scale);
}

void conv3x3(int64_t mode, const Tensor& X, int64_t x_bstride, int64_t x_off, int64_t x_ld, int64_t B, int64_t H,
             int64_t W, int64_t Cin, const Tensor& Wt, int64_t Nout, Tensor& out, int64_t out_ld, int64_t out_gap,
             int64_t out_off, int64_t accumulate) {
    check_gpu(X, "X", false); check_gpu(Wt, "Wt"); check_gpu(out, "out", false);
    TORCH_CHECK(X.scalar_type() == Wt.scalar_type(), "conv3x3: X and Wt dtypes differ");
    c10::DeviceGuard g(X.device());
    DCLIP_CALL(dclip_conv3x3((int)mode, dt_code(X.scalar_type()), X.data_ptr(), x_bstride, x_off, x_ld, (int)B, (int)H,
                             (int)W, (int)Cin, Wt.data_ptr(), (int)Nout, out.data_ptr(), dt_code(out.scalar_type()), out_ld,
                             (int)out_gap, (int)out_off, (int)accumulate, stream_of(X)));
}

Tensor conv3x3_wgrad(const Tensor& dY, int64_t ldy, int64_t Nout, const Tensor& X, int64_t x_bstride, int64_t x_off,
                     int64_t x_ld, int64_t B, int64_t H, int64_t W, int64_t Cin, int64_t splits, bool oihw,
                     const c10::optional<Tensor>& scale) {
    check_gpu(dY, "dY", false); check_gpu(X, "X", false);
    TORCH_CHECK(oihw || !(scale.has_value() && scale->defined()), "conv3x3_wgrad: a scale needs the OIHW output");
    c10::DeviceGuard g(X.device());
    Tensor dW = oihw ? at::empty({Nout, Cin, 3, 3}, like(X, at::kFloat)) : at::empty({Nout, 9 * Cin}, like(X, at::kFloat));
    Tensor ws = at::empty({splits * Nout * 9 * Cin}, like(X, at::kFloat));
    DCLIP_CALL(dclip_conv3x3_wgrad(dt_code(dY.scalar_type()), dY.data_ptr(), ldy, (int)Nout, X.data_ptr(), x_bstride,
                                   x_off, x_ld, (int)B, (int)H, (int)W, (int)Cin, ptr<float>(dW), ws.data_ptr(),
                                   (int)splits, oihw ? 1 : 0, scale_entry(scale, 1), stream_of(X)));
    return dW;
}

int lab_code(at::ScalarType t) {
    switch (t) {
        case at::kLong: return 0;
        case at::kInt: return 1;
        case at::kByte: return 2;
        default: TORCH_CHECK(false, "upsample_ce: labels must be int64, int32 or uint8");
    }
    return -1;
}

std::tuple<Tensor, Tensor, Tensor> upsample_ce(const Tensor& logits, const Tensor& labels, int64_t ignore_index) {
    check_gpu(logits, "logits"); check_gpu(labels, "labels");
    TORCH_CHECK(logits.dim() == 4 && labels.dim() == 3 && labels.size(0) == logits.size(0), "upsample_ce: shapes");
    c10::DeviceGuard g(logits.device());
    Tensor sums = at::zeros({1}, like(logits, at::kDouble));
    Tensor cnt = at::zeros({1}, like(logits, at::kInt));
    Tensor grad = at::zeros(logits.sizes(), like(logits, at::kFloat));
    Tensor ws = at::empty({dclip_upsample_ws_floats((int)logits.size(0), (int)logits.size(1), (int)logits.size(2),
                                                    (int)logits.size(3))}, like(logits, at::kFloat));
    DCLIP_CALL(dclip_upsample_ce(dt_code(logits.scalar_type()), logits.data_ptr(), (int)logits.size(0),
                                 (int)logits.size(1), (int)logits.size(2), (int)logits.size(3), labels.data_ptr(),
                                 lab_code(labels.scalar_type()), (int)labels.size(1), (int)labels.size(2),
                                 (int)ignore_index, (double*)sums.data_ptr(), (unsigned*)cnt.data_ptr(), ptr<float>(grad),
                                 ptr<float>(ws), stream_of(logits)));
    return {sums, cnt, grad};
}

Tensor upsample_silog_sums(const Tensor& pred, const Tensor& target, const c10::optional<Tensor>& mask, double eps) {
    check_gpu(pred, "pred"); check_gpu(target, "target"); check_opt(mask, "mask");
    TORCH_CHECK(target.scalar_type() == at::kFloat && target.dim() == 3, "upsample_silog: target (B, H, W) fp32");
    c10::DeviceGuard g(pred.device());
    Tensor sums = at::zeros({3}, like(pred, at::kDouble));
    Tensor ws = at::empty({dclip_upsample_ws_floats((int)pred.size(0), 1, (int)pred.size(2), (int)pred.size(3))},
                          like(pred, at::kFloat));
    DCLIP_CALL(dclip_upsample_silog(0, dt_code(pred.scalar_type()), pred.data_ptr(), (int)pred.size(0), (int)pred.size(2),
                                    (int)pred.size(3), ptr<float>(target), optr<uint8_t>(mask), (int)target.size(1),
                                    (int)target.size(2), (float)eps, 0.f, (double*)sums.data_ptr(), nullptr,
                                    ptr<float>(ws), stream_of(pred)));
    return sums;
}

Tensor upsample_silog_grad(const Tensor& pred, const Tensor& target, const c10::optional<Tensor>& mask,
                           const Tensor& sums, double eps, double lambd) {
    check_gpu(pred, "pred"); check_gpu(target, "target"); check_opt(mask, "mask"); check_gpu(sums, "sums");
    c10::DeviceGuard g(pred.device());
    Tensor grad = at::zeros(pred.sizes(), like(pred, at::kFloat));
    Tensor ws = at::empty({dclip_upsample_ws_floats((int)pred.size(0), 1, (int)pred.size(2), (int)pred.size(3))},
                          like(pred, at::kFloat));
    DCLIP_CALL(dclip_upsample_silog(1, dt_code(pred.scalar_type()), pred.data_ptr(), (int)pred.size(0), (int)pred.size(2),
                                    (int)pred.size(3), ptr<float>(target), optr<uint8_t>(mask), (int)target.size(1),
                                    (int)target.size(2), (float)eps, (float)lambd, (double*)sums.data_ptr(),
                                    ptr<float>(grad), ptr<float>(ws), stream_of(pred)));
    return grad;
}

std::tuple<Tensor, Tensor, Tensor, Tensor> cityscapes_prepare(const Tensor& img, const Tensor& ids, const Tensor& disp,
// ... 628 lines not shown
    m.impl("gemm_gelu", &gemm_gelu);
    m.impl("gemm_gelu_h", &gemm_gelu_h);
    m.impl("gemm_residual_lp", &gemm_residual_lp);
    m.impl("weight_grad", &weight_grad);
    m.impl("gemm_tn", &gemm_tn);
    m.impl("cast", &cast);
    m.impl("grad_scale", &grad_scale);
    m.impl("row_scale_add", &row_scale_add);
    m.impl("bn_eval", &bn_eval);
    m.impl("transpose2d", &transpose2d);
    m.impl("weight_refresh", &weight_refresh);
    m.impl("transpose_batched", &transpose_batched);
    m.impl("add_readout_cast", &add_readout_cast);
    m.impl("add_readout_amax", &add_readout_amax);
    m.impl("add_readout_cast_scaled", &add_readout_cast_scaled);
    m.impl("layernorm_bwd_scaled", &layernorm_bwd_scaled);
    m.impl("layernorm_bwd_scaled_add", &layernorm_bwd_scaled_add);
    m.impl("attn_fwd", &attn_fwd);
    m.impl("attn_fwd_fp8", &attn_fwd_fp8);
    m.impl("attn_bwd", &attn_bwd);
    m.impl("attn_bwd_fp8", &attn_bwd_fp8);
    m.impl("im2col", &im2col);
    m.impl("tokens_fwd", &tokens_fwd);
    m.impl("tokens_bwd", &tokens_bwd);
    m.impl("pos_interp", &pos_interp);
    m.impl("pos_interp_bwd", &pos_interp_bwd);
    m.impl("row_mean", &row_mean);
    m.impl("score_map", &score_map);
    m.impl("score_concat", &score_concat);
    m.impl("bilinear", &bilinear);
    m.impl("bilinear_bwd", &bilinear_bwd);
    m.impl("bn_fwd", &bn_fwd);
    m.impl("bn_bwd", &bn_bwd);
    m.impl("bn_fwd_rows", &bn_fwd_rows);
    m.impl("bn_bwd_rows", &bn_bwd_rows);
    m.impl("conv3x3", &conv3x3);
    m.impl("conv3x3_wgrad", &conv3x3_wgrad);
    m.impl("upsample_ce", &upsample_ce);
    m.impl("upsample_silog_sums", &upsample_silog_sums);
    m.impl("upsample_silog_grad", &upsample_silog_grad);
    m.impl("cityscapes_prepare", &cityscapes_prepare);
}

TORCH_LIBRARY(dclip_eval, m) {
    m.def("upsample_argmax(Tensor logits, int H, int W) -> Tensor");
    m.def("seg_update(Tensor logits, Tensor labels, int ignore_index, Tensor(a!) cm, Tensor(b!) ce_sums, "
          "bool want_pred) -> Tensor?");
    m.def("depth_update(Tensor pred, Tensor target, Tensor? mask, float min_depth, float max_depth, bool clamp_pred, "
          "float eps, Tensor(a!) sums, bool want_up) -> Tensor?");
    m.def("ensemble_argmax(Tensor[] logits, int[] flips, int H, int W, bool probs) -> Tensor");
    m.def("ensemble_seg_update(Tensor[] logits, int[] flips, Tensor labels, int ignore_index, bool probs, "
          "Tensor(a!) cm, Tensor(b!) ce_sums, bool want_pred) -> Tensor?");
    m.def("ensemble_depth(Tensor[] preds, int[] flips, int H, int W) -> Tensor");
    m.def("ensemble_depth_update(Tensor[] preds, int[] flips, Tensor target, Tensor? mask, float min_depth, "
          "float max_depth, bool clamp_pred, float eps, Tensor(a!) sums, bool want_up) -> Tensor?");
    m.def("slide_argmax(Tensor[] logits, int[] origins, int wh, int ww, int H, int W) -> Tensor");
    m.def("slide_seg_update(Tensor[] logits, int[] origins, int wh, int ww, Tensor labels, int ignore_index, "
          "Tensor(a!) cm, Tensor(b!) ce_sums, bool want_pred) -> Tensor?");
    m.def("slide_depth(Tensor[] preds, int[] origins, int wh, int ww, int H, int W) -> Tensor");
    m.def("slide_depth_update(Tensor[] preds, int[] origins, int wh, int ww, Tensor target, Tensor? mask, "
          "float min_depth, float max_depth, bool clamp_pred, float eps, Tensor(a!) sums, bool want_up) -> Tensor?");
    m.def("slide_tta_argmax(Tensor[] logits, int[] views, int[] origins, int H, int W, bool probs) -> Tensor");
    m.def("slide_tta_seg_update(Tensor[] logits, int[] views, int[] origins, Tensor labels, int ignore_index, "
          "bool probs, Tensor(a!) cm, Tensor(b!) ce_sums, bool want_pred) -> Tensor?");
    m.def("slide_tta_depth(Tensor[] preds, int[] views, int[] origins, int H, int W) -> Tensor");
    m.def("slide_tta_depth_update(Tensor[] preds, int[] views, int[] origins, Tensor target, Tensor? mask, "
          "float min_depth, float max_depth, bool clamp_pred, float eps, Tensor(a!) sums, bool want_up) -> Tensor?");
    m.def("upsample_argmax_classes(Tensor logits, int H, int W) -> Tensor");
    m.def("seg_update_classes(Tensor logits, Tensor labels, int ignore_index, Tensor(a!) cm, Tensor(b!) ce_sums, "
          "bool want_pred, Tensor(c!)? ws=None) -> Tensor?");
    m.def("seg_classes_ws_bytes(int B, int K, int h, int w) -> int", &seg_classes_ws_bytes);
}

TORCH_LIBRARY(dclip_classes, m) {
    m.def("score_map(Tensor v, int bstride, int row_off, int ld, Tensor text, int B, int HW, float eps) -> Tensor");
    m.def("upsample_ce(Tensor logits, Tensor labels, int ignore_index) -> (Tensor, Tensor, Tensor)");
}

TORCH_LIBRARY_IMPL(dclip_classes, CUDA, m) {
    m.impl("score_map", &score_map_classes);
    m.impl("upsample_ce", &upsample_ce_classes);
}

TORCH_LIBRARY(dclip_loss, m) {
    m.def("upsample_ce(Tensor logits, Tensor labels, int ignore_index, Tensor? class_weight, float label_smoothing, "
          "Tensor? pixel_weight, bool want_pixel_loss, bool want_grad) -> "
          "(Tensor sums, Tensor count, Tensor? grad, Tensor? pixel_loss)");
}

TORCH_LIBRARY_IMPL(dclip_loss, CUDA, m) { m.impl("upsample_ce", &upsample_ce_opt); }

TORCH_LIBRARY_IMPL(dclip_eval, CUDA, m) {
    m.impl("upsample_argmax_classes", &upsample_argmax_classes);
    m.impl("seg_update_classes", &seg_update_classes);
    m.impl("slide_tta_argmax", &slide_tta_argmax);
    m.impl("slide_tta_seg_update", &slide_tta_seg_update);
    m.impl("slide_tta_depth", &slide_tta_depth);
    m.impl("slide_tta_depth_update", &slide_tta_depth_update);
    m.impl("upsample_argmax", &upsample_argmax);
    m.impl("seg_update", &seg_update);
    m.impl("depth_update", &depth_update);
    m.impl("ensemble_argmax", &ensemble_argmax);
    m.impl("ensemble_seg_update", &ensemble_seg_update);
    m.impl("ensemble_depth", &ensemble_depth);
    m.impl("ensemble_depth_update", &ensemble_depth_update);
    m.impl("slide_argmax", &slide_argmax);
    m.impl("slide_seg_update", &slide_seg_update);
    m.impl("slide_depth", &slide_depth);
    m.impl("slide_depth_update", &slide_depth_update);
}

TORCH_LIBRARY(dclip_optim, m) {
    m.def("adamw_prepare(Tensor desc, Tensor desc_host, Tensor[] grads, int tiles, Tensor hp, Tensor? found_inf, "
          "Tensor(a!) state, bool with_norm) -> ()");
    m.def("adamw_update(Tensor desc, Tensor desc_host, Tensor[] grads, int tiles, Tensor state) -> ()");
}

TORCH_LIBRARY_IMPL(dclip_optim, CUDA, m) {
    m.impl("adamw_prepare", &adamw_prepare);
    m.impl("adamw_update", &adamw_update);
}
```

denseclip_vit_multimodal_amd/ops.py:

```python
import math
import weakref

import torch

from . import _native as N

N_ = N

_DT = {torch.float32: N.F32, torch.float16: N.F16, torch.bfloat16: N.BF16}


def _dt(t):
    try:
        return _DT[t.dtype]
    except KeyError:
        raise TypeError(f"unsupported dtype {t.dtype}") from None


def _p(t):
    return None if t is None else t.data_ptr()


def _stream():
    return torch.cuda.current_stream().cuda_stream


TIMING = None
TIMING_OPS = False
STATS = {}


def _stat(name):
    STATS[name] = STATS.get(name, 0) + 1


def _tic():
    if TIMING is None:
        return None
    e = torch.cuda.Event(enable_timing=True)
    e.record()
    return e


def _toc(name, e0):
    if e0 is None:
        return
    e1 = torch.cuda.Event(enable_timing=True)
    e1.record()
    TIMING.setdefault(name, []).append((e0, e1))


def timing_summary():
    torch.cuda.synchronize()
    out = {}
    for k, evs in (TIMING or {}).items():
        tot = sum(a.elapsed_time(b) for a, b in evs)
        out[k] = (len(evs), tot, tot / max(1, len(evs)))
    return out


def _check(*ts, strided=()):
    for t in ts + tuple(strided):
        if t is None:
            continue
        if not t.is_cuda:
            raise RuntimeError("denseclip HIP op got a CPU tensor: the MI355X path has no CPU fallback")
    for t in ts:
        if t is not None and not t.is_contiguous():
            raise RuntimeError("denseclip HIP op needs contiguous tensors")


_D = None


class _TimedOps:

    def __init__(self, d):
        self._d = d

    def __getattr__(self, name):
        fn = getattr(self._d, name)

        def call(*a, **k):
            e0 = _tic()
            r = fn(*a, **k)
            _toc("op:" + name, e0)
            return r
        return call


from ._native import CLASSES_MAX


def DC():
    D()
    return torch.ops.dclip_classes


def DL():
    D()
    return torch.ops.dclip_loss


def D():
    global _D
    if _D is None:
        from . import _torch_ops
        _D = _torch_ops.load()
    if TIMING_OPS and TIMING is not None:
        return _TimedOps(_D)
    return _D


def _env_option(opt, default=0):
    import os
    for kv in filter(None, os.environ.get("DCLIP_OPTIONS", "").split(",")):
        k, v = kv.split("=")
        if int(k) == opt:
            return int(v)
    return default


_GEMM_WALK = [_env_option(N.OPT_GEMM_SCHED)]


def set_gemm_walk(walk):
    prev = _GEMM_WALK[0]
    if walk != prev:
        N.call("dclip_set_option", N.OPT_GEMM_SCHED, int(walk))
        _GEMM_WALK[0] = int(walk)
    return prev


def layernorm_fwd(x2d, w, b, out_dtype, eps=1e-5):
    _check(x2d, w, b)
    return D().layernorm_fwd(x2d, w, b, out_dtype, float(eps))


def layernorm_bwd(dy, x, w, mean, rstd, dw, db, res=None, lp_dtype=None, dy_scale=None, dy_ntok=0):
    _check(dy, x, w, mean, rstd, dw, db, res, dy_scale)
    if lp_dtype is None:
        return D().layernorm_bwd(dy, x, w, mean, rstd, res, dw, db, dy_scale, int(dy_ntok))
    assert dy_ntok == 0
    return D().layernorm_bwd_lp(dy, x, w, mean, rstd, res, dw, db, lp_dtype, dy_scale)


def layernorm_bwd_add(dy, x, w, mean, rstd, dw, db, res, add, ntok, lp_dtype):
    _check(dy, x, w, mean, rstd, dw, db, res, add)
    e0 = _tic()
    out = D().layernorm_bwd_add(dy, x, w, mean, rstd, res, add, ntok, dw, db, lp_dtype)
    _toc("layernorm_bwd_add", e0)
    return out


FOLD_READOUT_GRAD = True


class ReadoutLink:
    __slots__ = ("gh", "gw", "g", "lp", "ds", "hsb", "pair")

    def __init__(self, gh, gw, ds=None, hsb=None):
        self.gh, self.gw, self.ds, self.hsb = gh, gw, ds, hsb
        self.g = self.lp = self.pair = None


def gemm(A, B, epi=N.EPI_STORE, bias=None, aux=None, out_dtype=None, alpha=1.0, scale=None, lp_copy=False):
    _check(A, B, bias, aux, scale)
    assert A.shape[1] == B.shape[1], (A.shape, B.shape)
    e0 = _tic()
    if lp_copy:
        assert epi == N.EPI_RESIDUAL and alpha == 1.0 and scale is None and out_dtype in (None, torch.float32)
        out = D().gemm_residual_lp(A, B, bias, aux)
    elif epi == N.EPI_GELU:
        out = D().gemm_gelu(A, B, bias)
    else:
        odt = out_dtype or (torch.float32 if epi == N.EPI_RESIDUAL else A.dtype)
        out = D().gemm(A, B, epi, bias, aux, odt, float(alpha), scale)
    _toc("gemm", e0)
    return out
# ... 915 lines not shown
                   (xr.storage_offset() if xr is xmap else 0), xr is xmap)
        ctx.cdt = cdt
        ctx.hsb = _head_scale_buf()
        _stat("conv3x3")
        y = out.as_strided((B, Cout, H, W), (H * W * cp, 1, W * cp, cp))
        return y

    @staticmethod
    def backward(ctx, dy):
        xr, weight = ctx.saved_tensors
        B, Cin, H, W, Cout, cp, bs, ld, in_dt, in_strides, _, in_place = ctx.geo
        cdt = ctx.cdt
        M = B * H * W
        dyr = torch.zeros(M, cp, dtype=cdt, device=dy.device)
        dyr[:, :Cout] = dy.permute(0, 2, 3, 1).reshape(M, Cout)
        dx = dw = None
        if ctx.needs_input_grad[0]:
            w_t = _conv3x3_dgrad_rows(weight, cdt)
            if in_place and in_strides[0] == bs:
                gap_rows = (bs - H * W * ld) // ld
                buf = torch.empty(B * bs, dtype=cdt, device=dy.device)
                D().conv3x3(1, dyr, H * W * cp, 0, cp, B, H, W, cp, w_t, Cin, buf, ld, gap_rows, gap_rows, 0)
                dx = buf.as_strided((B, Cin, H, W), (bs, 1, W * ld, ld), gap_rows * ld)
            else:
                buf = torch.empty(M, Cin, dtype=cdt, device=dy.device)
                D().conv3x3(1, dyr, H * W * cp, 0, cp, B, H, W, cp, w_t, Cin, buf, Cin, 0, 0, 0)
                dx = buf.as_strided((B, Cin, H, W), (H * W * Cin, 1, W * Cin, Cin))
            if in_dt != cdt:
                dx = dx.to(in_dt)
        if ctx.needs_input_grad[1]:
            tiles = (cp + 127) // 128 * (9 * Cin // 128)
            splits = max(1, min(32, 512 // max(1, tiles), M // 4096 or 1))
            e0 = _tic()
            dw = D().conv3x3_wgrad(dyr, cp, cp, xr, bs, 0, ld, B, H, W, Cin, splits, True, ctx.hsb)
            _toc("conv_wgrad", e0)
            dw = dw[:Cout]
            if dw.dtype != weight.dtype:
                dw = dw.to(weight.dtype)
        return dx, dw, None


def _conv3x3_rows(weight, cdt):
    Cout, Cin = weight.shape[:2]
    cp = _pad64(Cout)

    def rows(w):
        if cp == Cout and w.is_cuda:
            return D().transpose_batched(w.contiguous(), Cout, Cin, 9, 9, Cin, cdt).view(Cout, 9 * Cin)
        r = w.permute(0, 2, 3, 1).reshape(Cout, 9 * Cin)
        return torch.cat([r, r.new_zeros(cp - Cout, 9 * Cin)]) if cp > Cout else r
    return WEIGHTS.get_with(weight, cdt, "conv3x3_rows", rows)


def _conv3x3_dgrad_rows(weight, cdt):
    Cout, Cin = weight.shape[:2]
    cp = _pad64(Cout)
    if cp == Cout and weight.is_cuda:
        return WEIGHTS.get(weight, cdt, transposed=True).view(Cin, 9 * cp)

    def trows(w):
        t = w.permute(1, 2, 3, 0)
        if cp > Cout:
            t = torch.cat([t, t.new_zeros(Cin, 3, 3, cp - Cout)], dim=3)
        return t.reshape(Cin, 9 * cp)
    return WEIGHTS.get_with(weight, cdt, "conv3x3_dgrad", trows)


class NeckLevelsFn(torch.autograd.Function):

    @staticmethod
    def forward(ctx, meta, *args):
        bns, cdt = meta
        L = len(bns)
        maps = args[:L]
        convw = args[L:2 * L]
        bnw = args[2 * L:3 * L]
        bnb = args[3 * L:4 * L]
        B, Cin, H, W = maps[0].shape
        Ci = convw[0].shape[0]
        M, LC = B * H * W, L * Ci
        pre = torch.empty(M, LC, dtype=cdt, device=maps[0].device)
        out = torch.empty(M, LC, dtype=cdt, device=maps[0].device)
        geo, stats = [], []
        for l in range(L):
            xr, bs, ld = pixel_rows(maps[l], cdt)
            D().conv3x3(0, xr, bs, 0, ld, B, H, W, Cin, _conv3x3_rows(convw[l], cdt), Ci, pre[:, l * Ci:], LC, 0, 0, 0)
            bn = bns[l]
            if bn.num_batches_tracked is not None:
                bn.num_batches_tracked.add_(1)
            mean, rstd = D().bn_fwd_rows(pre[:, l * Ci:(l + 1) * Ci], bnw[l].detach(), bnb[l].detach(), bn.running_mean,
                                         bn.running_var, float(bn.momentum), float(bn.eps), True,
                                         out[:, l * Ci:(l + 1) * Ci])
            geo.append((xr, bs, ld))
            stats += [mean, rstd]
        ctx.save_for_backward(pre, *[g[0] for g in geo], *convw, *bnw, *bnb, *stats)
        ctx.meta = (L, B, Cin, H, W, Ci, cdt, [(g[1], g[2]) for g in geo], [m.dtype for m in maps],
                    [tuple(m.stride()) for m in maps], [g[0] is m for g, m in zip(geo, maps)])
        ctx.hsb = _head_scale_buf()
        ctx.links = [getattr(m, "_dclip_link", None) for m in maps]
        _stat("neck_levels")
        return out.as_strided((B, LC, H, W), (H * W * LC, 1, W * LC, LC))

    @staticmethod
    def backward(ctx, dout):
        L, B, Cin, H, W, Ci, cdt, bsld, in_dts, in_strides, in_place = ctx.meta
        saved = ctx.saved_tensors
        pre = saved[0]
        xrs = saved[1:1 + L]
        convw = saved[1 + L:1 + 2 * L]
        bnw = saved[1 + 2 * L:1 + 3 * L]
        bnb = saved[1 + 3 * L:1 + 4 * L]
        stats = saved[1 + 4 * L:]
        M, LC = B * H * W, L * Ci
        d = dout.to(cdt).permute(0, 2, 3, 1).reshape(M, LC)
        if not d.is_contiguous():
            d = d.contiguous()
        dpre = torch.empty(M, LC, dtype=cdt, device=d.device)
        need = ctx.needs_input_grad
        dmaps, dconv, dbnw, dbnb = [None] * L, [None] * L, [None] * L, [None] * L
        tiles = (Ci + 127) // 128 * (9 * Cin // 128)
        splits = max(1, min(32, 512 // max(1, tiles), M // 4096 or 1))
        for l in range(L):
            sl = slice(l * Ci, (l + 1) * Ci)
            dbnw[l], dbnb[l] = D().bn_bwd_rows(d[:, sl], pre[:, sl], bnw[l].detach(), bnb[l].detach(), stats[2 * l],
                                               stats[2 * l + 1], True, True, True, dpre[:, sl], ctx.hsb)
            bs, ld = bsld[l]
            if need[1 + l]:
                w_t = _conv3x3_dgrad_rows(convw[l], cdt)
                if in_place[l] and in_strides[l][0] == bs:
                    gap_rows = (bs - H * W * ld) // ld
                    buf = torch.empty(B * bs, dtype=cdt, device=d.device)
                    D().conv3x3(1, dpre[:, l * Ci:], H * W * LC, 0, LC, B, H, W, Ci, w_t, Cin, buf, ld, gap_rows,
                                gap_rows, 0)
                    dm = buf.as_strided((B, Cin, H, W), (bs, 1, W * ld, ld), gap_rows * ld)
                else:
                    buf = torch.empty(M, Cin, dtype=cdt, device=d.device)
                    D().conv3x3(1, dpre[:, l * Ci:], H * W * LC, 0, LC, B, H, W, Ci, w_t, Cin, buf, Cin, 0, 0, 0)
                    dm = buf.as_strided((B, Cin, H, W), (H * W * Cin, 1, W * Cin, Cin))
                dmaps[l] = dm if in_dts[l] == cdt else dm.to(in_dts[l])
                if ctx.links[l] is not None:
                    ctx.links[l].g = dmaps[l]
            if need[1 + L + l]:
                e0 = _tic()
                dwc = D().conv3x3_wgrad(dpre[:, l * Ci:], LC, Ci, xrs[l], bs, 0, ld, B, H, W, Cin, splits, True, ctx.hsb)
                _toc("conv_wgrad", e0)
                dconv[l] = dwc if dwc.dtype == convw[l].dtype else dwc.to(convw[l].dtype)
        return (None, *dmaps, *dconv, *dbnw, *dbnb)


def neck_levels_hip_ok(layers, feats):
    if not feats or not all(f.is_cuda and f.dim() == 4 and f.dtype in (torch.bfloat16, torch.float16) for f in feats):
        return False
    if len({(tuple(f.shape), f.dtype) for f in feats}) != 1:
        return False
    Ci = layers[0][0].weight.shape[0]
    for layer in layers:
        conv, bn = layer[0], layer[1]
        if conv.kernel_size != (3, 3) or conv.bias is not None or conv.weight.shape[0] != Ci or \
                not conv3x3_supported(feats[0], conv.weight):
            return False
        f32 = all(t is not None and t.dtype == torch.float32 for t in (bn.weight, bn.bias, bn.running_mean,
                                                                       bn.running_var))
        if not (bn.training and bn.track_running_stats and bn.momentum is not None and f32):
            return False
    return Ci % 64 == 0 and len(layers) * Ci <= 2048


def conv3x3_supported(xmap, weight):
    return (xmap.is_cuda and xmap.dim() == 4 and weight.shape[2:] == (3, 3) and xmap.shape[1] % 128 == 0
            and weight.shape[1] == xmap.shape[1])


class Conv1x1Fn(torch.autograd.Function):

    @staticmethod
    def forward(ctx, xmap, weight, bias, cdt):
        B, Cin, H, W = xmap.shape
        Cout = weight.shape[0]
        x2 = xmap.to(cdt).permute(0, 2, 3, 1).reshape(B * H * W, Cin).contiguous()
        out = gemm(x2, WEIGHTS.get(weight, cdt), bias=bias.detach() if bias is not None else None)
        ctx.save_for_backward(x2, weight)
        ctx.meta = (B, Cin, H, W, Cout, bias is not None, xmap.dtype)
        ctx.cdt = cdt
        ctx.hsb = _head_scale_buf()
        _stat("conv1x1")
        return out.as_strided((B, Cout, H, W), (H * W * Cout, 1, W * Cout, Cout))

    @staticmethod
    def backward(ctx, dy):
        x2, weight = ctx.saved_tensors
        B, Cin, H, W, Cout, has_b, in_dt = ctx.meta
        cdt = ctx.cdt
        d2 = dy.permute(0, 2, 3, 1).reshape(B * H * W, Cout)
        d2 = d2.to(cdt).contiguous()
        dx = dw = db = None
        if ctx.needs_input_grad[0]:
            dx = gemm(d2, WEIGHTS.get(weight, cdt, transposed=True))
            dx = dx.as_strided((B, Cin, H, W), (H * W * Cin, 1, W * Cin, Cin))
            if in_dt != cdt:
                dx = dx.to(in_dt)
        if ctx.needs_input_grad[1] or (has_b and ctx.needs_input_grad[2]):
            dWm, dbm = weight_grad(d2, x2, want_bias=has_b, scale=ctx.hsb)
            dw = dWm.view_as(weight).to(weight.dtype)
            db = dbm
        return dx, dw, db, None


def conv1x1_supported(xmap, weight):
# ... 235 lines not shown
```

include/dclip.h:

```cpp
#ifndef DCLIP_H
#define DCLIP_H

#include <stdint.h>

#ifdef __cplusplus
extern "C" {
#endif

#define DCLIP_F32 0
#define DCLIP_F16 1
#define DCLIP_BF16 2
#define DCLIP_U8 3

#define DCLIP_OK 0
#define DCLIP_ERR_ARG (-1)
#define DCLIP_ERR_HIP (-2)

#define DCLIP_EPI_STORE 0
#define DCLIP_EPI_GELU 1
#define DCLIP_EPI_RESIDUAL 2
#define DCLIP_EPI_GELU_BWD 3
#define DCLIP_EPI_SPLITK 4
#define DCLIP_EPI_STORE_SCALED 5

const char* dclip_last_error(void);
int dclip_abi_version(void);

#define DCLIP_OPT_ATTN_FWD_WAVES 0
#define DCLIP_OPT_ATTN_DQ_WAVES 1
#define DCLIP_OPT_ATTN_DKDV_WAVES 2
#define DCLIP_OPT_GEMM_TILE 3
#define DCLIP_OPT_GEMM_TN_TILE 4
#define DCLIP_OPT_ATTN_DKDV_QS 5
#define DCLIP_OPT_ATTN_BWD_KERNEL 7
#define DCLIP_OPT_ATTN_FWD_KERNEL 6
#define DCLIP_OPT_ATTN_BWD_BLOCK 8
#define DCLIP_OPT_GEMM_TN_COLSUM 9
#define DCLIP_OPT_GEMM_EPI 10
#define DCLIP_OPT_GEMM_TAIL 11
#define DCLIP_OPT_ATTN_FP8_QK 12
#define DCLIP_OPT_ATTN_DQ_ISSUE 13
#define DCLIP_OPT_ATTN_DQ_ROWS 14
#define DCLIP_OPT_ATTN_DQ_DEFER 15
#define DCLIP_OPT_GEMM_SCHED 16
#define DCLIP_OPT_GEMM_KLOOP 17
#define DCLIP_OPT_ATTN_DQ_REDUCE 18
#define DCLIP_OPT_ATTN_PREP_ORDER 19
#define DCLIP_OPT_ATTN_BWD_WGS 20
#define DCLIP_OPT_COUNT 21
int dclip_set_option(int id, int value);

int dclip_layernorm_fwd(const void* x, int x_dt, const float* w, const float* b,
                        void* y, int y_dt, float* mean, float* rstd,
                        int64_t rows, int64_t cols, float eps, void* stream);

int dclip_layernorm_bwd(const void* dy, int dy_dt, const void* x, int x_dt,
                        const float* w, const float* mean, const float* rstd,
                        float* dx, int accumulate, float* dw, float* db,
                        int64_t rows, int64_t cols, void* stream);
int dclip_layernorm_bwd_res(const void* dy, int dy_dt, const float* dy_scale, int64_t dy_ntok,
                            const void* x, int x_dt, const float* w, const float* mean, const float* rstd,
                            const float* res, float* dx, void* lp, int lp_dt, float* dw, float* db,
                            float* ws, int64_t rows, int64_t cols, void* stream);
int64_t dclip_layernorm_bwd_ws_floats(int64_t rows, int64_t cols);

int dclip_gemm(int epilogue, int ab_dt,
               const void* A, int64_t lda, const void* B, int64_t ldb,
               int64_t M, int64_t N, int64_t K, int splits, float alpha, const float* alpha_ptr,
               const float* bias, const void* aux, int aux_dt, int64_t ld_aux,
               void* C, int c_dt, int64_t ldc, void* C2, int64_t ldc2, void* stream);

int dclip_gemm_tn_plan(int64_t M, int64_t N, int64_t K, int* splits, int64_t* K_pad);

int dclip_gemm_tn(int epilogue, int ab_dt, const void* A, int64_t lda, const void* B, int64_t ldb,
                  int64_t M, int64_t N, int64_t K, int64_t K_pad, int splits, float alpha,
                  const float* alpha_ptr, const float* bias,
                  void* ws, void* C, int64_t ldc, float* colsum_a, void* stream);

int dclip_attn_fwd(int dt, const void* qkv, void* o, float* lse,
                   int B, int N, int H, int D, float scale, void* stream);

int dclip_attn_bwd(int dt, const void* qkv, const void* o, const void* dout,
                   const float* lse, float* delta_ws, void* dqkv,
                   int B, int N, int H, int D, float scale, void* stream);

int64_t dclip_attn_bwd_fp8_workspace(int B, int N, int H);
int dclip_attn_bwd_fp8(int dt, const void* qkv, const void* o, const void* dout, const float* lse, float* ws,
                       void* dqkv, int B, int N, int H, int D, float scale, void* stream);
int64_t dclip_attn_bwd_workspace(int B, int N, int H);

int dclip_attn_fwd_fp8(int dt, const void* qkv, void* o, float* lse, void* ws,
                       int B, int N, int H, int D, void* stream);
int64_t dclip_attn_fwd_fp8_workspace(int B, int N, int H);

int dclip_im2col(const void* img, int img_dt, void* out, int out_dt, int64_t ldo,
                 int B, int Cin, int Hin, int Win, int p, void* stream);

int dclip_tokens_fwd(const void* patch, int patch_dt, const float* cls, const float* pos,
                     float* x, int B, int P, int C, void* stream);

int dclip_tokens_bwd(const float* dx, void* dpatch, int dpatch_dt, float dpatch_scale,
                     const float* dpatch_scale_ptr, float* dcls, float* dpos, int B, int P, int C,
                     void* stream);

int dclip_pos_interp_fwd(const float* pos, float* out, int g, int C, int H, int W,
                         void* stream);
int dclip_pos_interp_bwd(const float* dout, float* dpos, int g, int C, int H, int W,
                         void* stream);

int dclip_transpose(const void* in, int in_dt, int64_t in_bstride, int64_t in_ld, int64_t r0,
                    void* out, int out_dt, int64_t out_bstride, int64_t out_ld,
                    int batch, int64_t rows, int64_t rows_pad, int64_t cols,
                    int accumulate, float* colsum, void* stream);

int dclip_weight_refresh(const int64_t* desc, int n, int64_t tiles, int out_dt, void* stream);

int64_t dclip_row_mean_workspace(int B, int64_t rows, int C);
int dclip_row_mean(const void* x, int x_dt, int64_t bstride, int64_t row_off, int64_t ld, int B, int64_t rows,
                   int C, float* ws, float* out, void* stream);

int dclip_score_map(const void* v, int v_dt, int64_t bstride, int64_t row_off, int64_t ld, const float* t,
                    float* score, int B, int HW, int C, int K, float eps, void* stream);

int dclip_score_concat(const void* rows, int dt, int64_t bstride, int64_t row_off, int64_t ld, int C,
                       const float* score, int K, int hs, int ws, void* out, int B, int h, int w, void* stream);

int dclip_bilinear_fwd(const void* in, int in_dt, void* out, int out_dt,
                       int64_t NC, int Hi, int Wi, int Ho, int Wo, void* stream);
int dclip_bilinear_bwd(const void* dout, int dout_dt, float* din, float* ws,
                       int64_t NC, int Hi, int Wi, int Ho, int Wo, void* stream);

int dclip_conv3x3(int mode, int ab_dt, const void* X, int64_t x_bstride, int64_t x_off, int64_t x_ld,
// ... 55 lines not shown
typedef struct {
    const void* low;
    int y0, x0;
} dclip_window;
int64_t dclip_slide_eval_ws_bytes(int B, int K, int nwin);
int dclip_slide_eval_seg(int low_dt, const dclip_window* wins, int nwin, int B, int K, int h, int w, int wh, int ww,
                         const void* labels, int lab_dt, int H, int W, int ignore_index, uint8_t* pred, int64_t* cm,
                         double* loss_sum, unsigned long long* count, void* ws, void* stream);
int dclip_slide_eval_depth(int low_dt, const dclip_window* wins, int nwin, int B, int h, int w, int wh, int ww,
                           const float* target, const uint8_t* mask, int H, int W, float min_depth, float max_depth,
                           int clamp_pred, float eps, float* up, double* sums, void* ws, void* stream);

#define DCLIP_SLIDE_TTA_MAX_WINDOWS 1024
typedef struct {
    int Hv, Wv, flip, wh, ww, h, w, first, nwin;
} dclip_slide_view;
int64_t dclip_slide_tta_eval_ws_bytes(int B, int K, int nviews, int nwin_total);
int dclip_slide_tta_eval_seg(int low_dt, const dclip_slide_view* views, int nviews, const dclip_window* wins,
                             int nwin_total, int B, int K, int average, const void* labels, int lab_dt, int H, int W,
                             int ignore_index, uint8_t* pred, int64_t* cm, double* loss_sum,
                             unsigned long long* count, void* ws, void* stream);
int dclip_slide_tta_eval_depth(int low_dt, const dclip_slide_view* views, int nviews, const dclip_window* wins,
                               int nwin_total, int B, const float* target, const uint8_t* mask, int H, int W,
                               float min_depth, float max_depth, int clamp_pred, float eps, float* up, double* sums,
                               void* ws, void* stream);

int dclip_cityscapes_prepare(const uint8_t* img, const uint8_t* ids, const uint16_t* disp, int B, int H, int W,
                             const int* crop, int h, int w, const float* mean, const float* stdv, float bf,
                             float depth_max, void* out_img, int out_dt, int64_t* out_seg, float* out_depth,
                             uint8_t* out_mask, void* stream);

int dclip_cityscapes_augment(const uint8_t* img, const uint8_t* ids, const uint16_t* disp, int B, int H, int W,
                             const int* params, int h, int w, const float* mean, const float* stdv, float bf,
                             float depth_max, void* out_img, int out_dt, int64_t* out_seg, float* out_depth,
                             uint8_t* out_mask, void* stream);

int dclip_color_jitter(uint8_t* img, int B, int h, int w, const double* params, unsigned long long* ws,
                       void* stream);

int dclip_normalize_u8(const uint8_t* img, int B, int h, int w, const float* mean, const float* stdv, void* out,
                       int out_dt, void* stream);

int dclip_cast(const void* in, int in_dt, void* out, int out_dt, int64_t n, float scale,
               const float* scale_ptr, void* stream);

int dclip_bn_eval(int dt, const void* x, int64_t rows, int C, int64_t ld, const float* w, const float* b, float eps,
                  const float* running_mean, const float* running_var, float* ws, void* y, int relu, void* stream);

int dclip_row_scale_add(const float* x, const float* y, const float* s, int ntok, float* out, int64_t rows,
                        int cols, void* stream);

int dclip_grad_scale(const float* g, int64_t n, float target, float* ws, void* stream);
int dclip_add_readout_cast(const float* a, const void* b, int b_dt, float* sum, void* lp, int lp_dt,
                           int64_t rows, int cols, int ntok, float scale, void* stream);

int dclip_add_readout_amax(const float* a, const void* b, int b_dt, const float* b_scale_ptr, float* sum,
                           int64_t rows, int cols, int ntok, float target, float* ws, void* stream);

#define DCLIP_DS_STATE_FLOATS 196
int dclip_add_readout_cast_scaled(const float* a, const void* b, int b_dt, const float* b_scale_ptr, float* sum,
                                  void* lp, int64_t rows, int cols, int ntok, float target, float* st, int use,
                                  float* spair, void* stream);
int dclip_layernorm_bwd_scaled(const void* dy, int dy_dt, const float* dy_scale, const void* x, int x_dt,
                               const float* w, const float* mean, const float* rstd, const float* res, float* dx,
                               void* lp, float* dw, float* db, float* ws, int64_t rows, int64_t cols, float target,
                               float* st, int use, float* spair, void* stream);

int dclip_layernorm_bwd_add(const void* dy, int dy_dt, const float* x, const float* w, const float* mean,
                            const float* rstd, const float* res, const void* add, int ntok, float* dx, void* lp,
                            int lp_dt, float* dw, float* db, float* ws, int64_t rows, int64_t cols, void* stream);
int dclip_layernorm_bwd_scaled_add(const void* dy, int dy_dt, const float* dy_scale, const float* x,
                                   const float* w, const float* mean, const float* rstd, const float* res,
                                   const void* add, int add_dt, const float* add_scale, int ntok, float* dx,
                                   void* lp, float* dw, float* db, float* ws, int64_t rows, int64_t cols,
                                   float target, float* st, int use, float* spair, void* stream);

int64_t dclip_bn_workspace(int64_t rows, int C);
int dclip_bn_fwd(int dt, const void* x, int64_t rows, int C, int64_t ld, const float* w, const float* b,
                 float eps, float momentum, float* running_mean, float* running_var, float* ws, float* mean,
                 float* rstd, void* y, int relu, void* stream);
int dclip_bn_bwd(int dt, const void* dy, const void* x, int64_t rows, int C, int64_t ld, const float* w,
                 const float* b, const float* mean, const float* rstd, float* ws, void* dx, float* dw,
                 float* db, int relu, const float* gscale, void* stream);

#define DCLIP_ADAMW_DESC_WORDS 12
#define DCLIP_ADAMW_CHUNK 256
#define DCLIP_ADAMW_HP_FLOATS 8
#define DCLIP_ADAMW_STATE_HEAD 8
#define DCLIP_ADAMW_STATE_ROW_FLOATS 12
int64_t dclip_adamw_ws_bytes(int64_t tiles);
int dclip_adamw_prepare(const int64_t* desc, const int64_t* desc_host, const void* const* grads, int n,
                        int64_t tiles, const float* hp, int n_rows, const float* found_inf, float* state,
                        void* ws, int with_norm, void* stream);
int dclip_adamw_update(const int64_t* desc, const int64_t* desc_host, const void* const* grads, int n,
                       int64_t tiles, float* state, void* stream);

#ifdef __cplusplus
}
#endif
#endif
```

Measured before the change: 62.99.

## Batch neck BatchNorm levels into single launches and fold GEMM tail into persistent kernel

Adds multi-level BatchNorm forward/backward kernels that process all FPN neck levels in one launch, indexing per-level weights and running stats through a pointer table and blockIdx.y. This replaces a per-level loop of BN stats, finalize and apply launches, and moves the num_batches_tracked increment onto the device. Separately, the 16-row GEMM tail is now computed by extra workgroups appended to the persistent GEMM grid instead of a second kernel launch, so the tail can overlap the main tiles. The cost is more complex launch plumbing and a tail path that shares shared memory with the persistent kernel.

After: 63.42 (median of 6 runs). No clear change (+0.7%).

```diff
diff --git a/denseclip_vit_multimodal_amd/_native.py b/denseclip_vit_multimodal_amd/_native.py
--- a/denseclip_vit_multimodal_amd/_native.py
+++ b/denseclip_vit_multimodal_amd/_native.py
@@ -14,6 +14,7 @@
 OPT_ATTN_DQ_REDUCE = 18
 OPT_ATTN_PREP_ORDER = 19
 OPT_ATTN_BWD_WGS = 20
+OPT_BN_LEVELS = 21
 OPT_ATTN_DQ_DEFER = 15
 
 _c_void_p = ctypes.c_void_p
@@ -86,6 +87,11 @@
                      _c_void_p, _c_void_p, _c_void_p, _c_void_p, _i32, _c_void_p],
     "dclip_bn_bwd": [_i32, _c_void_p, _c_void_p, _i64, _i32, _i64, _c_void_p, _c_void_p, _c_void_p, _c_void_p,
                      _c_void_p, _c_void_p, _c_void_p, _c_void_p, _i32, _c_void_p, _c_void_p],
+    "dclip_bn_levels_workspace": [_i64, _i32, _i32],
+    "dclip_bn_fwd_levels": [_i32, _c_void_p, _i64, _i32, _i32, _i64, _c_void_p, _c_void_p, _f32, _f32, _c_void_p,
+                            _c_void_p, _c_void_p, _c_void_p, _c_void_p, _c_void_p, _c_void_p, _i32, _c_void_p],
+    "dclip_bn_bwd_levels": [_i32, _c_void_p, _c_void_p, _i64, _i32, _i32, _i64, _c_void_p, _c_void_p, _c_void_p,
+                            _c_void_p, _c_void_p, _c_void_p, _c_void_p, _c_void_p, _i32, _c_void_p, _c_void_p],
     "dclip_conv3x3": [_i32, _i32, _c_void_p, _i64, _i64, _i64, _i32, _i32, _i32, _i32, _c_void_p, _i32, _c_void_p,
                       _i32, _i64, _i32, _i32, _i32, _c_void_p],
     "dclip_upsample_ce": [_i32, _c_void_p, _i32, _i32, _i32, _i32, _c_void_p, _i32, _i32, _i32, _i32, _c_void_p,
@@ -208,6 +214,7 @@
         lib.dclip_attn_bwd_workspace.restype = ctypes.c_int64
         lib.dclip_attn_bwd_fp8_workspace.restype = ctypes.c_int64
         lib.dclip_bn_workspace.restype = ctypes.c_int64
+        lib.dclip_bn_levels_workspace.restype = ctypes.c_int64
         lib.dclip_attn_fwd_fp8_workspace.restype = ctypes.c_int64
         lib.dclip_row_mean_workspace.restype = ctypes.c_int64
         lib.dclip_layernorm_bwd_ws_floats.restype = ctypes.c_int64
diff --git a/denseclip_vit_multimodal_amd/_torch_ops.py b/denseclip_vit_multimodal_amd/_torch_ops.py
--- a/denseclip_vit_multimodal_amd/_torch_ops.py
+++ b/denseclip_vit_multimodal_amd/_torch_ops.py
@@ -317,6 +317,14 @@
                 _e(*logits.shape, like=logits, dtype=f32) if want_grad else None,
                 _e(*labels.shape, like=logits, dtype=f32) if want_pixel_loss else None)
 
+    @reg("dclip_neck::bn_levels_fwd")
+    def _(x, w, b, running_mean, running_var, num_batches_tracked, momentum, eps, relu, y):
+        return _e(x.shape[1], like=x, dtype=f32), _e(x.shape[1], like=x, dtype=f32)
+
+    @reg("dclip_neck::bn_levels_bwd")
+    def _(dy, x, w, b, mean, rstd, relu, dx, scale=None):
+        return _e(x.shape[1], like=x, dtype=f32), _e(x.shape[1], like=x, dtype=f32)
+
     @reg("dclip_optim::adamw_prepare")
     def _(desc, desc_host, grads, tiles, hp, found_inf, state, with_norm):
         return None
diff --git a/denseclip_vit_multimodal_amd/csrc/gemm.hip b/denseclip_vit_multimodal_amd/csrc/gemm.hip
--- a/denseclip_vit_multimodal_amd/csrc/gemm.hip
+++ b/denseclip_vit_multimodal_amd/csrc/gemm.hip
@@ -825,12 +825,21 @@
     return ntiles;
 }
 
+template <typename T, int EPI, typename OutT, int NWAVES>
+__device__ __forceinline__ void tail16x16_unit(const T* __restrict__ A, int64_t lda, const T* __restrict__ B,
+                                               int64_t ldb, int mt, int W, int IT, int m0, int n0,
+                                               const float* __restrict__ bias, const void* __restrict__ aux,
+                                               int64_t ld_aux, void* __restrict__ C, int64_t ldc,
+                                               void* __restrict__ C2, int64_t ldc2, Alpha alpha_arg,
+                                               float (*__restrict__ red)[16][17]);
+
 template <typename T, int EPI, typename OutT, int NW = 8, bool ELDS = false, bool DYN = false, bool NTS = false,
           bool PF = false>
 __global__ __launch_bounds__(64 * NW, 1) void gemm_nt_pers_kernel(
     const T* __restrict__ A, int64_t lda, const T* __restrict__ B, int64_t ldb, int K, int tiles_m, int tiles_n,
     const float* __restrict__ bias, const void* __restrict__ aux, int64_t ld_aux, void* __restrict__ C, int64_t ldc,
-    void* __restrict__ C2, int64_t ldc2, Alpha alpha_arg, unsigned* __restrict__ sched = nullptr) {
+    void* __restrict__ C2, int64_t ldc2, Alpha alpha_arg, unsigned* __restrict__ sched = nullptr, int mt = 0,
+    int tail_w = 0, int tail_it = 0) {
     const float alpha = alpha_arg.get();
     typedef BigCfg<256, 256, 2, NW / 2, 2, 64> Cfg;
     typedef typename Mfma<T>::frag frag;
@@ -842,10 +851,17 @@
     constexpr bool epi_lds = NW == 8 && ELDS;
     const int l16 = lane & 15, lq = lane >> 4;
     const int ntiles = tiles_m * tiles_n;
-    const int G = gridDim.x;
+    const int G = (int)gridDim.x - (mt > 0 ? 16 * tiles_n : 0);
+    const int M = tiles_m * 256, N = tiles_n * 256;
+    if ((int)blockIdx.x >= G) {
+        static_assert(sizeof(float) * 16 * 16 * 17 <= Cfg::SMEM, "the tail's partial sums fit the staging ring");
+        tail16x16_unit<T, EPI, OutT, NW>(A + (int64_t)M * lda, lda, B, ldb, mt, tail_w, tail_it, M,
+                                         ((int)blockIdx.x - G) * 16, bias, aux, ld_aux, C, ldc, C2, ldc2, alpha_arg,
+                                         (float(*)[16][17])smem);
+        return;
+    }
     const int r = xcd_remap(blockIdx.x, G);
     const int nk = K / 64;
-    const int M = tiles_m * 256, N = tiles_n * 256;
 
     const uint32_t abytes = (uint32_t)((int64_t)M * lda * sizeof(T)), bbytes = (uint32_t)((int64_t)N * ldb * sizeof(T));
     const uint32_t lda_b = (uint32_t)(lda * sizeof(T)), ldb_b = (uint32_t)(ldb * sizeof(T));
@@ -1897,19 +1913,17 @@
     }
 }
 
-template <typename T, int EPI, typename OutT>
-__global__ __launch_bounds__(1024) void gemm_tail16x16_kernel(const T* __restrict__ A, int64_t lda,
-                                                              const T* __restrict__ B, int64_t ldb, int mt, int N,
-                                                              int W, int IT, int m0, const float* __restrict__ bias,
-                                                              const void* __restrict__ aux, int64_t ld_aux,
-                                                              void* __restrict__ C, int64_t ldc, void* __restrict__ C2,
-                                                              int64_t ldc2, Alpha alpha_arg) {
+template <typename T, int EPI, typename OutT, int NWAVES>
+__device__ __forceinline__ void tail16x16_unit(const T* __restrict__ A, int64_t lda, const T* __restrict__ B,
+                                               int64_t ldb, int mt, int W, int IT, int m0, int n0,
+                                               const float* __restrict__ bias, const void* __restrict__ aux,
+                                               int64_t ld_aux, void* __restrict__ C, int64_t ldc,
+                                               void* __restrict__ C2, int64_t ldc2, Alpha alpha_arg,
+                                               float (*__restrict__ red)[16][17]) {
     typedef typename Mfma<T>::frag frag;
-    constexpr int ITMAX = 6;
-    __shared__ float red[16][16][17];
+    constexpr int ITMAX = 6, SPW = 16 / NWAVES;
     const int lane = threadIdx.x & 63, wave = threadIdx.x >> 6;
     const int l16 = lane & 15, lq = lane >> 4;
-    const int n0 = blockIdx.x * 16;
     const int t = threadIdx.x;
     const int er = t >> 1, ecb = (t & 1) * 8;
     const bool epi = t < 2 * mt;
@@ -1925,26 +1939,34 @@
         if constexpr (EPI == DCLIP_EPI_GELU_BWD) load8<T>((const T*)aux + (int64_t)(m0 + er) * ld_aux + nb, pre, true, 8);
     }
     const bool rowok = l16 < mt;
-    const int kbeg = wave * IT * 32;
-    const T* arow = A + (int64_t)(rowok ? l16 : 0) * lda + kbeg + 8 * lq;
-    const T* brow = B + (int64_t)(n0 + l16) * ldb + kbeg + 8 * lq;
     frag zf;
 #pragma unroll
     for (int j = 0; j < 8; ++j) zf[j] = (T)0.f;
-    frag a[ITMAX], b[ITMAX];
-#pragma unroll
-    for (int it = 0; it < ITMAX; ++it) {
-        if (it < IT) {
-            a[it] = rowok ? *(const frag*)(arow + 32 * it) : zf;
-            b[it] = *(const frag*)(brow + 32 * it);
-        }
-    }
-    f32x4 acc = f32x4{0.f, 0.f, 0.f, 0.f};
-#pragma unroll
-    for (int it = 0; it < ITMAX; ++it)
-        if (it < IT) acc = Mfma16<T>::mma(a[it], b[it], acc);
-#pragma unroll
-    for (int e = 0; e < 4; ++e) red[wave][4 * lq + e][l16] = acc[e];
+    frag a[SPW][ITMAX], b[SPW][ITMAX];
+#pragma unroll
+    for (int s = 0; s < SPW; ++s) {
+        const int kbeg = (wave + NWAVES * s) * IT * 32;
+        const T* arow = A + (int64_t)(rowok ? l16 : 0) * lda + kbeg + 8 * lq;
+        const T* brow = B + (int64_t)(n0 + l16) * ldb + kbeg + 8 * lq;
+#pragma unroll
+        for (int it = 0; it < ITMAX; ++it) {
+            if (it < IT && wave + NWAVES * s < W) {
+                a[s][it] = rowok ? *(const frag*)(arow + 32 * it) : zf;
+                b[s][it] = *(const frag*)(brow + 32 * it);
+            }
+        }
+    }
+#pragma unroll
+    for (int s = 0; s < SPW; ++s) {
+        if (wave + NWAVES * s < W) {
+            f32x4 acc = f32x4{0.f, 0.f, 0.f, 0.f};
+#pragma unroll
+            for (int it = 0; it < ITMAX; ++it)
+                if (it < IT) acc = Mfma16<T>::mma(a[s][it], b[s][it], acc);
+#pragma unroll
+            for (int e = 0; e < 4; ++e) red[wave + NWAVES * s][4 * lq + e][l16] = acc[e];
+        }
+    }
     __syncthreads();
     if (epi) {
         const float alpha = alpha_arg.get();
@@ -1983,6 +2005,18 @@
             store8<OutT>((OutT*)C + m * ldc + nb, v, true, 8);
         }
     }
+}
+
+template <typename T, int EPI, typename OutT>
+__global__ __launch_bounds__(1024) void gemm_tail16x16_kernel(const T* __restrict__ A, int64_t lda,
+                                                              const T* __restrict__ B, int64_t ldb, int mt, int N,
+                                                              int W, int IT, int m0, const float* __restrict__ bias,
+                                                              const void* __restrict__ aux, int64_t ld_aux,
+                                                              void* __restrict__ C, int64_t ldc, void* __restrict__ C2,
+                                                              int64_t ldc2, Alpha alpha_arg) {
+    __shared__ float red[16][16][17];
+    tail16x16_unit<T, EPI, OutT, 16>(A, lda, B, ldb, mt, W, IT, m0, blockIdx.x * 16, bias, aux, ld_aux, C, ldc, C2, ldc2,
+                                     alpha_arg, red);
 }
 
 inline bool tail16x16_plan(int64_t K, int& W, int& IT) {
@@ -2137,15 +2171,18 @@
             return false;
         const int tail_opt = dclip_option(DCLIP_OPT_GEMM_TAIL);
         int tw = 0, tit = 0;
-        if (tail > 0 && tail <= 16 && tail_opt == 0 && tail16x16_plan(K, tw, tit)) {
+        const bool t16 = tail > 0 && tail <= 16 && (tail_opt == 0 || tail_opt == 3) && tail16x16_plan(K, tw, tit);
+        const int fold_mt = (t16 && tail_opt == 0 && !PIPE) ? (int)tail : 0;
+        const unsigned fold_wgs = fold_mt > 0 ? (unsigned)(N / 16) : 0u;
+        if (t16 && fold_mt == 0) {
             gemm_tail16x16_kernel<T, EPI, OutT><<<(unsigned)(N / 16), 64 * tw, 0, st>>>(
                 (const T*)A + Mfull * lda, lda, (const T*)B, ldb, (int)tail, (int)N, tw, tit, (int)Mfull, bias, aux,
                 ld_aux, C, ldc, C2, ldc2, alpha);
-        } else if (tail > 0 && tail <= 16 && K % 256 == 0 && tail_opt != 1) {
+        } else if (fold_mt == 0 && tail > 0 && tail <= 16 && K % 256 == 0 && tail_opt != 1) {
             gemm_tail16_kernel<T, EPI, OutT><<<(unsigned)(N / 64), 512, 0, st>>>(
                 (const T*)A + Mfull * lda, lda, (const T*)B, ldb, (int)tail, (int)N, (int)K, (int)Mfull, bias, aux,
                 ld_aux, C, ldc, C2, ldc2, alpha);
-        } else if (tail > 0) {
+        } else if (fold_mt == 0 && tail > 0) {
             const int tiles_n = (int)(N / 256);
             const int ksteps = (int)(K / 64);
             int ts = 1;
@@ -2174,13 +2211,13 @@
                                   ? gemm_sched_counters(st)
                                   : nullptr;
             if (sched != nullptr)
-                gemm_nt_pers_kernel<T, EPI, OutT, NW, true, NW == 8><<<G, 64 * NW, 0, st>>>(
+                gemm_nt_pers_kernel<T, EPI, OutT, NW, true, NW == 8><<<G + fold_wgs, 64 * NW, 0, st>>>(
                     (const T*)A, lda, (const T*)B, ldb, (int)K, (int)(Mfull / 256), (int)(N / 256), bias, aux, ld_aux, C,
-                    ldc, C2, ldc2, alpha, sched);
+                    ldc, C2, ldc2, alpha, sched, fold_mt, tw, tit);
 #define PERS_LAUNCH(NTS_, PF_)                                                                                  \
-    gemm_nt_pers_kernel<T, EPI, OutT, NW, true, false, NTS_, PF_><<<G, 64 * NW, 0, st>>>(                        \
+    gemm_nt_pers_kernel<T, EPI, OutT, NW, true, false, NTS_, PF_><<<G + fold_wgs, 64 * NW, 0, st>>>(             \
         (const T*)A, lda, (const T*)B, ldb, (int)K, (int)(Mfull / 256), (int)(N / 256), bias, aux, ld_aux, C, ldc, C2, \
-        ldc2, alpha)
+        ldc2, alpha, nullptr, fold_mt, tw, tit)
             else if (NW == 8 && dclip_option(DCLIP_OPT_GEMM_EPI) != 1) {
                 const bool nts = pers_streaming_stores(EPI, N), pf = pers_prefetch_kloop(EPI);
                 if (nts && pf) PERS_LAUNCH(true, true);
@@ -2190,9 +2227,9 @@
             }
 #undef PERS_LAUNCH
             else
-                gemm_nt_pers_kernel<T, EPI, OutT, NW, false><<<G, 64 * NW, 0, st>>>(
+                gemm_nt_pers_kernel<T, EPI, OutT, NW, false><<<G + fold_wgs, 64 * NW, 0, st>>>(
                     (const T*)A, lda, (const T*)B, ldb, (int)K, (int)(Mfull / 256), (int)(N / 256), bias, aux, ld_aux, C,
-                    ldc, C2, ldc2, alpha);
+                    ldc, C2, ldc2, alpha, nullptr, fold_mt, tw, tit);
         }
         return true;
     }
diff --git a/denseclip_vit_multimodal_amd/csrc/misc.hip b/denseclip_vit_multimodal_amd/csrc/misc.hip
--- a/denseclip_vit_multimodal_amd/csrc/misc.hip
+++ b/denseclip_vit_multimodal_amd/csrc/misc.hip
@@ -1000,6 +1000,16 @@
     return (int)(need < BN_NBLK_MAX ? need : BN_NBLK_MAX);
 }
 
+constexpr int BN_LEVELS_MAX = 16;
+struct BnLevels {
+    const float* w[BN_LEVELS_MAX];
+    const float* b[BN_LEVELS_MAX];
+    float* rmean[BN_LEVELS_MAX];
+    float* rvar[BN_LEVELS_MAX];
+    long long* nbt[BN_LEVELS_MAX];
+    int64_t ws_stride;
+};
+
 template <typename T>
 __device__ __forceinline__ void load8(const T* p, float* v) {
     typedef T t8 __attribute__((ext_vector_type(8)));
@@ -1019,10 +1029,20 @@
 
 template <typename T, int MODE, bool RELU>
 __global__ void __launch_bounds__(256) bn_stats_kernel(const T* __restrict__ a, const T* __restrict__ x,
-                                                       const float* __restrict__ w, const float* __restrict__ b,
                                                        const float* __restrict__ mean, const float* __restrict__ rstd,
-                                                       int64_t rows, int C, int64_t ld, float* __restrict__ part) {
+                                                       int64_t rows, int C, int64_t ld, float* __restrict__ part,
+                                                       const BnLevels lv) {
     __shared__ float red[2 * 2048];
+    const int lev = blockIdx.y;
+    const float* __restrict__ w = lv.w[lev];
+    const float* __restrict__ b = lv.b[lev];
+    a += lev * C;
+    part += lev * lv.ws_stride;
+    if (MODE == 1) {
+        x += lev * C;
+        mean += lev * C;
+        rstd += lev * C;
+    }
     const int tpr = C / 8, rpb = 256 / tpr;
     const int c8 = threadIdx.x % tpr, rr = threadIdx.x / tpr;
     float s[8], q[8], ref[8], sc[8], sh[8];
@@ -1100,12 +1120,22 @@
 
 template <typename T>
 __global__ void bn_fwd_finalize_kernel(const float* __restrict__ part, int nblk, const T* __restrict__ x, int64_t rows,
-                                       int C, const float* __restrict__ w, const float* __restrict__ b, float eps,
-                                       float momentum, float* __restrict__ rmean, float* __restrict__ rvar,
-                                       float* __restrict__ mean, float* __restrict__ rstd, float* __restrict__ ss) {
+                                       int C, float eps, float momentum, float* __restrict__ mean,
+                                       float* __restrict__ rstd, float* __restrict__ ss, const BnLevels lv) {
+    const int lev = blockIdx.y;
+    const float* __restrict__ w = lv.w[lev];
+    const float* __restrict__ b = lv.b[lev];
+    float* __restrict__ rmean = lv.rmean[lev];
+    float* __restrict__ rvar = lv.rvar[lev];
+    part += lev * lv.ws_stride;
+    ss += lev * lv.ws_stride;
+    x += lev * C;
+    mean += lev * C;
+    rstd += lev * C;
     int c;
     float S, Q;
     bn_reduce_parts(part, nblk, C, c, S, Q);
+    if (blockIdx.x == 0 && threadIdx.x == 0 && lv.nbt[lev] != nullptr) *lv.nbt[lev] += 1;
     if (threadIdx.x >= 8 || c >= C) return;
     const float n = (float)rows;
     const float md = S / n;
@@ -1124,9 +1154,17 @@
 }
 
 __global__ void bn_bwd_finalize_kernel(const float* __restrict__ part, int nblk, int64_t rows, int C,
-                                       const float* __restrict__ w, const float* __restrict__ mean,
-                                       const float* __restrict__ rstd, float* __restrict__ dw, float* __restrict__ db,
-                                       float* __restrict__ k, const float* __restrict__ gscale) {
+                                       const float* __restrict__ mean, const float* __restrict__ rstd,
+                                       float* __restrict__ dw, float* __restrict__ db, float* __restrict__ k,
+                                       const float* __restrict__ gscale, const BnLevels lv) {
+    const int lev = blockIdx.y;
+    const float* __restrict__ w = lv.w[lev];
+    part += lev * lv.ws_stride;
+    k += lev * lv.ws_stride;
+    mean += lev * C;
+    rstd += lev * C;
+    if (dw) dw += lev * C;
+    if (db) db += lev * C;
     int c;
     float S, Q;
     bn_reduce_parts(part, nblk, C, c, S, Q);
@@ -1145,7 +1183,11 @@
 template <typename T, bool BWD, bool RELU>
 __global__ void __launch_bounds__(256) bn_apply_kernel(const T* __restrict__ a, const T* __restrict__ x,
                                                        const float* __restrict__ k, int64_t rows, int C, int64_t ld,
-                                                       T* __restrict__ y) {
+                                                       T* __restrict__ y, int64_t ws_stride) {
+    a += blockIdx.y * C;
+    if (BWD) x += blockIdx.y * C;
+    y += blockIdx.y * C;
+    k += blockIdx.y * ws_stride;
     const int c8n = C / 8;
     const int64_t n8 = rows * c8n;
     typedef T t8 __attribute__((ext_vector_type(8)));
@@ -1174,9 +1216,14 @@
     }
 }
 
-__global__ void bn_mask_affine_kernel(const float* __restrict__ w, const float* __restrict__ b,
-                                      const float* __restrict__ mean, const float* __restrict__ rstd, int C,
-                                      float* __restrict__ k) {
+__global__ void bn_mask_affine_kernel(const float* __restrict__ mean, const float* __restrict__ rstd, int C,
+                                      float* __restrict__ k, const BnLevels lv) {
+    const int lev = blockIdx.y;
+    const float* __restrict__ w = lv.w[lev];
+    const float* __restrict__ b = lv.b[lev];
+    mean += lev * C;
+    rstd += lev * C;
+    k += lev * lv.ws_stride;
     const int c = blockIdx.x * 256 + threadIdx.x;
     if (c >= C) return;
     const float sc = (w ? w[c] : 1.f) * rstd[c];
@@ -1206,6 +1253,77 @@
     return (int64_t)BN_NBLK_MAX * 2 * C + 5 * (int64_t)C;
 }
 
+extern "C" int64_t dclip_bn_levels_workspace(int64_t rows, int L, int C) { return L * dclip_bn_workspace(rows, C); }
+
+namespace {
+
+int bn_fwd_run(int dt, const void* x, int64_t rows, int L, int C, int64_t ld, float eps, float momentum,
+               float* ws, float* mean, float* rstd, void* y, int relu, const BnLevels& lv, hipStream_t st) {
+    const int nblk = bn_nblk(rows, C);
+    float* ss = ws + (int64_t)BN_NBLK_MAX * 2 * C;
+    const unsigned ga = grid_for(rows * (C / 8), 8192);
+    const dim3 gs(nblk, L), gf((C + 7) / 8, L), gap(ga, L);
+#define BN_FWD(T)                                                                                                      \
+    bn_stats_kernel<T, 0, false><<<gs, 256, 0, st>>>((const T*)x, nullptr, nullptr, nullptr, rows, C, ld, ws, lv);     \
+    bn_fwd_finalize_kernel<T><<<gf, 256, 0, st>>>(ws, nblk, (const T*)x, rows, C, eps, momentum, mean, rstd, ss, lv);  \
+    if (relu)                                                                                                          \
+        bn_apply_kernel<T, false, true><<<gap, 256, 0, st>>>((const T*)x, nullptr, ss, rows, C, ld, (T*)y, lv.ws_stride); \
+    else                                                                                                               \
+        bn_apply_kernel<T, false, false><<<gap, 256, 0, st>>>((const T*)x, nullptr, ss, rows, C, ld, (T*)y, lv.ws_stride);
+    if (dt == DCLIP_BF16) {
+        BN_FWD(bf16)
+    } else {
+        BN_FWD(f16)
+    }
+#undef BN_FWD
+    DCLIP_LAUNCH_CHECK();
+    return 0;
+}
+
+int bn_bwd_run(int dt, const void* dy, const void* x, int64_t rows, int L, int C, int64_t ld, const float* mean,
+               const float* rstd, float* ws, void* dx, float* dw, float* db, int relu, const float* gscale,
+               const BnLevels& lv, hipStream_t st) {
+    const int nblk = bn_nblk(rows, C);
+    float* k = ws + (int64_t)BN_NBLK_MAX * 2 * C;
+    const unsigned ga = grid_for(rows * (C / 8), 8192);
+    const dim3 gs(nblk, L), gf((C + 7) / 8, L), gap(ga, L);
+    if (relu) bn_mask_affine_kernel<<<dim3((C + 255) / 256, L), 256, 0, st>>>(mean, rstd, C, k, lv);
+#define BN_BWD(T)                                                                                                      \
+    if (relu) {                                                                                                        \
+        bn_stats_kernel<T, 1, true><<<gs, 256, 0, st>>>((const T*)dy, (const T*)x, mean, rstd, rows, C, ld, ws, lv);   \
+        bn_bwd_finalize_kernel<<<gf, 256, 0, st>>>(ws, nblk, rows, C, mean, rstd, dw, db, k, gscale, lv);              \
+        bn_apply_kernel<T, true, true><<<gap, 256, 0, st>>>((const T*)dy, (const T*)x, k, rows, C, ld, (T*)dx,         \
+                                                            lv.ws_stride);                                             \
+    } else {                                                                                                           \
+        bn_stats_kernel<T, 1, false><<<gs, 256, 0, st>>>((const T*)dy, (const T*)x, mean, rstd, rows, C, ld, ws, lv);  \
+        bn_bwd_finalize_kernel<<<gf, 256, 0, st>>>(ws, nblk, rows, C, mean, rstd, dw, db, k, gscale, lv);              \
+        bn_apply_kernel<T, true, false><<<gap, 256, 0, st>>>((const T*)dy, (const T*)x, k, rows, C, ld, (T*)dx,        \
+                                                             lv.ws_stride);                                            \
+    }
+    if (dt == DCLIP_BF16) {
+        BN_BWD(bf16)
+    } else {
+        BN_BWD(f16)
+    }
+#undef BN_BWD
+    DCLIP_LAUNCH_CHECK();
+    return 0;
+}
+
+BnLevels bn_one_level(const float* w, const float* b, float* rmean, float* rvar, long long* nbt) {
+    BnLevels lv = {};
+    lv.w[0] = w;
+    lv.b[0] = b;
+    lv.rmean[0] = rmean;
+    lv.rvar[0] = rvar;
+    lv.nbt[0] = nbt;
+    return lv;
+}
+
+bool bn_levels_ok(int L, int C, int64_t ld) { return L >= 1 && L <= BN_LEVELS_MAX && (int64_t)L * C <= ld; }
+
+}
+
 extern "C" int dclip_bn_fwd(int dt, const void* x, int64_t rows, int C, int64_t ld, const float* w, const float* b,
                             float eps, float momentum, float* running_mean, float* running_var, float* ws, float* mean,
                             float* rstd, void* y, int relu, void* stream) {
@@ -1213,25 +1331,43 @@
     DCLIP_HOST_CHECK(bn_shape_ok(rows, C, ld), "dclip_bn_fwd: need rows > 0, C %% 8 == 0, C <= 2048, ld >= C, "
                      "ld %% 8 == 0 (C = %d)", C);
     DCLIP_HOST_CHECK(((uintptr_t)x % 16) == 0 && ((uintptr_t)y % 16) == 0, "dclip_bn_fwd: unaligned buffers");
-    hipStream_t st = (hipStream_t)stream;
-    const int nblk = bn_nblk(rows, C);
-    float* ss = ws + (int64_t)BN_NBLK_MAX * 2 * C;
-    const unsigned ga = grid_for(rows * (C / 8), 8192);
-#define BN_FWD(T)                                                                                                      \
-    bn_stats_kernel<T, 0, false><<<nblk, 256, 0, st>>>((const T*)x, nullptr, nullptr, nullptr, nullptr, nullptr, rows, \
-                                                       C, ld, ws);                                                     \
-    bn_fwd_finalize_kernel<T><<<(C + 7) / 8, 256, 0, st>>>(ws, nblk, (const T*)x, rows, C, w, b, eps, momentum,        \
-                                                           running_mean, running_var, mean, rstd, ss);                 \
-    if (relu) bn_apply_kernel<T, false, true><<<ga, 256, 0, st>>>((const T*)x, nullptr, ss, rows, C, ld, (T*)y);       \
-    else bn_apply_kernel<T, false, false><<<ga, 256, 0, st>>>((const T*)x, nullptr, ss, rows, C, ld, (T*)y);
-    if (dt == DCLIP_BF16) {
-        BN_FWD(bf16)
-    } else {
-        BN_FWD(f16)
-    }
-#undef BN_FWD
-    DCLIP_LAUNCH_CHECK();
-    return 0;
+    return bn_fwd_run(dt, x, rows, 1, C, ld, eps, momentum, ws, mean, rstd, y, relu,
+                      bn_one_level(w, b, running_mean, running_var, nullptr), (hipStream_t)stream);
+}
+
+extern "C" int dclip_bn_fwd_levels(int dt, const void* x, int64_t rows, int L, int C, int64_t ld, const float* const* w,
+                                   const float* const* b, float eps, float momentum, float* const* running_mean,
+                                   float* const* running_var, long long* const* num_batches_tracked, float* ws,
+                                   float* mean, float* rstd, void* y, int relu, void* stream) {
+    DCLIP_HOST_CHECK(dt == DCLIP_BF16 || dt == DCLIP_F16, "dclip_bn_fwd_levels: dtype must be bf16/f16");
+    DCLIP_HOST_CHECK(bn_shape_ok(rows, C, ld) && bn_levels_ok(L, C, ld),
+                     "dclip_bn_fwd_levels: need rows > 0, C %% 8 == 0, C <= 2048, 1 <= L <= %d, ld >= L * C, "
+                     "ld %% 8 == 0 (L = %d, C = %d)", BN_LEVELS_MAX, L, C);
+    DCLIP_HOST_CHECK(((uintptr_t)x % 16) == 0 && ((uintptr_t)y % 16) == 0, "dclip_bn_fwd_levels: unaligned buffers");
+    DCLIP_HOST_CHECK(w && b && running_mean && running_var && num_batches_tracked,
+                     "dclip_bn_fwd_levels: the pointer tables are required (their entries may be NULL)");
+    hipStream_t st = (hipStream_t)stream;
+    const int64_t stride = dclip_bn_workspace(rows, C);
+    if (dclip_option(DCLIP_OPT_BN_LEVELS) == 1) {
+        for (int l = 0; l < L; ++l) {
+            BnLevels lv = bn_one_level(w[l], b[l], running_mean[l], running_var[l], num_batches_tracked[l]);
+            const size_t off = (size_t)l * C * 2;
+            if (bn_fwd_run(dt, (const char*)x + off, rows, 1, C, ld, eps, momentum, ws + l * stride,
+                           mean + l * C, rstd + l * C, (char*)y + off, relu, lv, st) != 0)
+                return -1;
+        }
+        return 0;
+    }
+    BnLevels lv = {};
+    for (int l = 0; l < L; ++l) {
+        lv.w[l] = w[l];
+        lv.b[l] = b[l];
+        lv.rmean[l] = running_mean[l];
+        lv.rvar[l] = running_var[l];
+        lv.nbt[l] = num_batches_tracked[l];
+    }
+    lv.ws_stride = stride;
+    return bn_fwd_run(dt, x, rows, L, C, ld, eps, momentum, ws, mean, rstd, y, relu, lv, st);
 }
 
 extern "C" int dclip_bn_eval(int dt, const void* x, int64_t rows, int C, int64_t ld, const float* w, const float* b,
@@ -1246,9 +1382,9 @@
     float* ss = ws + (int64_t)BN_NBLK_MAX * 2 * C;
     const unsigned ga = grid_for(rows * (C / 8), 8192);
     bn_eval_affine_kernel<<<(C + 255) / 256, 256, 0, st>>>(w, b, running_mean, running_var, eps, C, ss);
-#define BN_EVAL(T)                                                                                                 \
-    if (relu) bn_apply_kernel<T, false, true><<<ga, 256, 0, st>>>((const T*)x, nullptr, ss, rows, C, ld, (T*)y);   \
-    else bn_apply_kernel<T, false, false><<<ga, 256, 0, st>>>((const T*)x, nullptr, ss, rows, C, ld, (T*)y);
+#define BN_EVAL(T)                                                                                                    \
+    if (relu) bn_apply_kernel<T, false, true><<<ga, 256, 0, st>>>((const T*)x, nullptr, ss, rows, C, ld, (T*)y, 0);   \
+    else bn_apply_kernel<T, false, false><<<ga, 256, 0, st>>>((const T*)x, nullptr, ss, rows, C, ld, (T*)y, 0);
     if (dt == DCLIP_BF16) {
         BN_EVAL(bf16)
     } else {
@@ -1267,28 +1403,38 @@
                      "ld %% 8 == 0 (C = %d)", C);
     DCLIP_HOST_CHECK(((uintptr_t)dy % 16) == 0 && ((uintptr_t)x % 16) == 0 && ((uintptr_t)dx % 16) == 0,
                      "dclip_bn_bwd: unaligned buffers");
-    hipStream_t st = (hipStream_t)stream;
-    const int nblk = bn_nblk(rows, C);
-    float* k = ws + (int64_t)BN_NBLK_MAX * 2 * C;
-    const unsigned ga = grid_for(rows * (C / 8), 8192);
-    if (relu) bn_mask_affine_kernel<<<(C + 255) / 256, 256, 0, st>>>(w, b, mean, rstd, C, k);
-#define BN_BWD(T)                                                                                                      \
-    if (relu) {                                                                                                        \
-        bn_stats_kernel<T, 1, true><<<nblk, 256, 0, st>>>((const T*)dy, (const T*)x, w, b, mean, rstd, rows, C, ld, ws); \
-        bn_bwd_finalize_kernel<<<(C + 7) / 8, 256, 0, st>>>(ws, nblk, rows, C, w, mean, rstd, dw, db, k, gscale);               \
-        bn_apply_kernel<T, true, true><<<ga, 256, 0, st>>>((const T*)dy, (const T*)x, k, rows, C, ld, (T*)dx);          \
-    } else {                                                                                                           \
-        bn_stats_kernel<T, 1, false><<<nblk, 256, 0, st>>>((const T*)dy, (const T*)x, w, b, mean, rstd, rows, C, ld,   \
-                                                           ws);                                                        \
-        bn_bwd_finalize_kernel<<<(C + 7) / 8, 256, 0, st>>>(ws, nblk, rows, C, w, mean, rstd, dw, db, k, gscale);               \
-        bn_apply_kernel<T, true, false><<<ga, 256, 0, st>>>((const T*)dy, (const T*)x, k, rows, C, ld, (T*)dx);         \
-    }
-    if (dt == DCLIP_BF16) {
-        BN_BWD(bf16)
-    } else {
-        BN_BWD(f16)
-    }
-#undef BN_BWD
-    DCLIP_LAUNCH_CHECK();
-    return 0;
-}
+    return bn_bwd_run(dt, dy, x, rows, 1, C, ld, mean, rstd, ws, dx, dw, db, relu, gscale,
+                      bn_one_level(w, b, nullptr, nullptr, nullptr), (hipStream_t)stream);
+}
+
+extern "C" int dclip_bn_bwd_levels(int dt, const void* dy, const void* x, int64_t rows, int L, int C, int64_t ld,
+                                   const float* const* w, const float* const* b, const float* mean, const float* rstd,
+                                   float* ws, void* dx, float* dw, float* db, int relu, const float* gscale,
+                                   void* stream) {
+    DCLIP_HOST_CHECK(dt == DCLIP_BF16 || dt == DCLIP_F16, "dclip_bn_bwd_levels: dtype must be bf16/f16");
+    DCLIP_HOST_CHECK(bn_shape_ok(rows, C, ld) && bn_levels_ok(L, C, ld),
+                     "dclip_bn_bwd_levels: need rows > 0, C %% 8 == 0, C <= 2048, 1 <= L <= %d, ld >= L * C, "
+                     "ld %% 8 == 0 (L = %d, C = %d)", BN_LEVELS_MAX, L, C);
+    DCLIP_HOST_CHECK(((uintptr_t)dy % 16) == 0 && ((uintptr_t)x % 16) == 0 && ((uintptr_t)dx % 16) == 0,
+                     "dclip_bn_bwd_levels: unaligned buffers");
+    DCLIP_HOST_CHECK(w && b, "dclip_bn_bwd_levels: the pointer tables are required (their entries may be NULL)");
+    hipStream_t st = (hipStream_t)stream;
+    const int64_t stride = dclip_bn_workspace(rows, C);
+    if (dclip_option(DCLIP_OPT_BN_LEVELS) == 1) {
+        for (int l = 0; l < L; ++l) {
+            const size_t off = (size_t)l * C * 2;
+            if (bn_bwd_run(dt, (const char*)dy + off, (const char*)x + off, rows, 1, C, ld, mean + l * C, rstd + l * C,
+                           ws + l * stride, (char*)dx + off, dw ? dw + l * C : nullptr, db ? db + l * C : nullptr, relu,
+                           gscale, bn_one_level(w[l], b[l], nullptr, nullptr, nullptr), st) != 0)
+                return -1;
+        }
+        return 0;
+    }
+    BnLevels lv = {};
+    for (int l = 0; l < L; ++l) {
+        lv.w[l] = w[l];
+        lv.b[l] = b[l];
+    }
+    lv.ws_stride = stride;
+    return bn_bwd_run(dt, dy, x, rows, L, C, ld, mean, rstd, ws, dx, dw, db, relu, gscale, lv, st);
+}
diff --git a/denseclip_vit_multimodal_amd/csrc/torch_ops.cpp b/denseclip_vit_multimodal_amd/csrc/torch_ops.cpp
--- a/denseclip_vit_multimodal_amd/csrc/torch_ops.cpp
+++ b/denseclip_vit_multimodal_amd/csrc/torch_ops.cpp
@@ -699,6 +699,64 @@
                                        const c10::optional<Tensor>& b, const Tensor& mean, const Tensor& rstd, bool relu,
                                        bool want_w, bool want_b, Tensor& dx, const c10::optional<Tensor>& scale) {
     return bn_bwd_into(dy, x, w, b, mean, rstd, relu, want_w, want_b, dx, scale);
+}
+
+template <typename P>
+std::vector<P*> level_ptrs(at::TensorList ts, size_t L, int64_t C, at::ScalarType st, const char* what) {
+    TORCH_CHECK(ts.size() == L, "dclip_neck: ", what, " needs one tensor per level");
+    std::vector<P*> p(L);
+    for (size_t l = 0; l < L; ++l) {
+        TORCH_CHECK(ts[l].is_cuda() && ts[l].is_contiguous() && ts[l].scalar_type() == st &&
+                        ts[l].numel() == (st == at::kLong ? 1 : C),
+                    "dclip_neck: ", what, "[", l, "] must be a contiguous GPU tensor of the level's size");
+        p[l] = (P*)ts[l].data_ptr();
+    }
+    return p;
+}
+
+std::tuple<Tensor, Tensor> bn_levels_fwd(const Tensor& x, at::TensorList w, at::TensorList b, at::TensorList running_mean,
+                                         at::TensorList running_var, at::TensorList num_batches_tracked, double momentum,
+                                         double eps, bool relu, Tensor& y) {
+    const Rows r = rows_of(x), ry = rows_of(y);
+    const size_t L = w.size();
+    TORCH_CHECK(L >= 1 && r.C % (int64_t)L == 0, "dclip_neck::bn_levels_fwd: the columns must split into the levels");
+    TORCH_CHECK(r.rows == ry.rows && r.C == ry.C && r.ld == ry.ld && x.scalar_type() == y.scalar_type(),
+                "dclip_neck::bn_levels_fwd: the output must match the input's rows, channels and pitch");
+    const int64_t C = r.C / (int64_t)L;
+    auto pw = level_ptrs<const float>(w, L, C, at::kFloat, "weight"), pb = level_ptrs<const float>(b, L, C, at::kFloat, "bias");
+    auto pm = level_ptrs<float>(running_mean, L, C, at::kFloat, "running_mean");
+    auto pv = level_ptrs<float>(running_var, L, C, at::kFloat, "running_var");
+    auto pn = level_ptrs<long long>(num_batches_tracked, L, C, at::kLong, "num_batches_tracked");
+    c10::DeviceGuard g(x.device());
+    Tensor ws = at::empty({dclip_bn_levels_workspace(r.rows, (int)L, (int)C)}, like(x, at::kFloat));
+    Tensor mean = at::empty({r.C}, like(x, at::kFloat)), rstd = at::empty({r.C}, like(x, at::kFloat));
+    DCLIP_CALL(dclip_bn_fwd_levels(dt_code(x.scalar_type()), x.data_ptr(), r.rows, (int)L, (int)C, r.ld, pw.data(),
+                                   pb.data(), (float)eps, (float)momentum, pm.data(), pv.data(), pn.data(),
+                                   ptr<float>(ws), ptr<float>(mean), ptr<float>(rstd), y.data_ptr(), relu ? 1 : 0,
+                                   stream_of(x)));
+    return {mean, rstd};
+}
+
+std::tuple<Tensor, Tensor> bn_levels_bwd(const Tensor& dy, const Tensor& x, at::TensorList w, at::TensorList b,
+                                         const Tensor& mean, const Tensor& rstd, bool relu, Tensor& dx,
+                                         const c10::optional<Tensor>& scale) {
+    const Rows r = rows_of(x), rd = rows_of(dy), rdx = rows_of(dx);
+    const size_t L = w.size();
+    TORCH_CHECK(L >= 1 && r.C % (int64_t)L == 0, "dclip_neck::bn_levels_bwd: the columns must split into the levels");
+    TORCH_CHECK(rd.rows == r.rows && rd.C == r.C && rd.ld == r.ld && rdx.ld == r.ld && rdx.rows == r.rows && rdx.C == r.C,
+                "dclip_neck::bn_levels_bwd: the tensors must share rows, channels and pitch");
+    TORCH_CHECK(dy.scalar_type() == x.scalar_type() && dx.scalar_type() == x.scalar_type(),
+                "dclip_neck::bn_levels_bwd: dtypes must match");
+    const int64_t C = r.C / (int64_t)L;
+    auto pw = level_ptrs<const float>(w, L, C, at::kFloat, "weight"), pb = level_ptrs<const float>(b, L, C, at::kFloat, "bias");
+    check_vec(mean, r.C, "mean"); check_vec(rstd, r.C, "rstd");
+    c10::DeviceGuard g(x.device());
+    Tensor ws = at::empty({dclip_bn_levels_workspace(r.rows, (int)L, (int)C)}, like(x, at::kFloat));
+    Tensor dw = at::empty({r.C}, like(x, at::kFloat)), db = at::empty({r.C}, like(x, at::kFloat));
+    DCLIP_CALL(dclip_bn_bwd_levels(dt_code(x.scalar_type()), dy.data_ptr(), x.data_ptr(), r.rows, (int)L, (int)C, r.ld,
+                                   pw.data(), pb.data(), ptr<float>(mean), ptr<float>(rstd), ptr<float>(ws), dx.data_ptr(),
+                                   ptr<float>(dw), ptr<float>(db), relu ? 1 : 0, scale_entry(scale, 1), stream_of(x)));
+    return {dw, db};
 }
 
 void conv3x3(int64_t mode, const Tensor& X, int64_t x_bstride, int64_t x_off, int64_t x_ld, int64_t B, int64_t H,
@@ -1493,6 +1551,18 @@
     m.impl("upsample_ce", &upsample_ce_classes);
 }
 
+TORCH_LIBRARY(dclip_neck, m) {
+    m.def("bn_levels_fwd(Tensor x, Tensor[] w, Tensor[] b, Tensor(a!)[] running_mean, Tensor(b!)[] running_var, "
+          "Tensor(c!)[] num_batches_tracked, float momentum, float eps, bool relu, Tensor(d!) y) -> (Tensor, Tensor)");
+    m.def("bn_levels_bwd(Tensor dy, Tensor x, Tensor[] w, Tensor[] b, Tensor mean, Tensor rstd, bool relu, "
+          "Tensor(a!) dx, Tensor? scale=None) -> (Tensor, Tensor)");
+}
+
+TORCH_LIBRARY_IMPL(dclip_neck, CUDA, m) {
+    m.impl("bn_levels_fwd", &bn_levels_fwd);
+    m.impl("bn_levels_bwd", &bn_levels_bwd);
+}
+
 TORCH_LIBRARY(dclip_loss, m) {
     m.def("upsample_ce(Tensor logits, Tensor labels, int ignore_index, Tensor? class_weight, float label_smoothing, "
           "Tensor? pixel_weight, bool want_pixel_loss, bool want_grad) -> "
diff --git a/denseclip_vit_multimodal_amd/ops.py b/denseclip_vit_multimodal_amd/ops.py
--- a/denseclip_vit_multimodal_amd/ops.py
+++ b/denseclip_vit_multimodal_amd/ops.py
@@ -95,6 +95,11 @@
 def DC():
     D()
     return torch.ops.dclip_classes
+
+
+def DN():
+    D()
+    return torch.ops.dclip_neck
 
 
 def DL():
@@ -1176,20 +1181,29 @@
         pre = torch.empty(M, LC, dtype=cdt, device=maps[0].device)
         out = torch.empty(M, LC, dtype=cdt, device=maps[0].device)
         geo, stats = [], []
+        fused = (L <= 16 and len({(float(bn.momentum), float(bn.eps)) for bn in bns}) == 1
+                 and all(bn.num_batches_tracked is not None for bn in bns))
         for l in range(L):
             xr, bs, ld = pixel_rows(maps[l], cdt)
             D().conv3x3(0, xr, bs, 0, ld, B, H, W, Cin, _conv3x3_rows(convw[l], cdt), Ci, pre[:, l * Ci:], LC, 0, 0, 0)
+            geo.append((xr, bs, ld))
+            if fused:
+                continue
             bn = bns[l]
             if bn.num_batches_tracked is not None:
                 bn.num_batches_tracked.add_(1)
             mean, rstd = D().bn_fwd_rows(pre[:, l * Ci:(l + 1) * Ci], bnw[l].detach(), bnb[l].detach(), bn.running_mean,
                                          bn.running_var, float(bn.momentum), float(bn.eps), True,
                                          out[:, l * Ci:(l + 1) * Ci])
-            geo.append((xr, bs, ld))
             stats += [mean, rstd]
+        if fused:
+            stats = list(DN().bn_levels_fwd(pre, [w.detach() for w in bnw], [b.detach() for b in bnb],
+                                            [bn.running_mean for bn in bns], [bn.running_var for bn in bns],
+                                            [bn.num_batches_tracked for bn in bns], float(bns[0].momentum),
+                                            float(bns[0].eps), True, out))
         ctx.save_for_backward(pre, *[g[0] for g in geo], *convw, *bnw, *bnb, *stats)
         ctx.meta = (L, B, Cin, H, W, Ci, cdt, [(g[1], g[2]) for g in geo], [m.dtype for m in maps],
-                    [tuple(m.stride()) for m in maps], [g[0] is m for g, m in zip(geo, maps)])
+                    [tuple(m.stride()) for m in maps], [g[0] is m for g, m in zip(geo, maps)], fused)
         ctx.hsb = _head_scale_buf()
         ctx.links = [getattr(m, "_dclip_link", None) for m in maps]
         _stat("neck_levels")
@@ -1197,7 +1211,7 @@
 
     @staticmethod
     def backward(ctx, dout):
-        L, B, Cin, H, W, Ci, cdt, bsld, in_dts, in_strides, in_place = ctx.meta
+        L, B, Cin, H, W, Ci, cdt, bsld, in_dts, in_strides, in_place, fused = ctx.meta
         saved = ctx.saved_tensors
         pre = saved[0]
         xrs = saved[1:1 + L]
@@ -1214,10 +1228,15 @@
         dmaps, dconv, dbnw, dbnb = [None] * L, [None] * L, [None] * L, [None] * L
         tiles = (Ci + 127) // 128 * (9 * Cin // 128)
         splits = max(1, min(32, 512 // max(1, tiles), M // 4096 or 1))
+        if fused:
+            dw, db = DN().bn_levels_bwd(d, pre, [w.detach() for w in bnw], [b.detach() for b in bnb], stats[0], stats[1],
+                                        True, dpre, ctx.hsb)
+            dbnw, dbnb = list(dw.split(Ci)), list(db.split(Ci))
         for l in range(L):
             sl = slice(l * Ci, (l + 1) * Ci)
-            dbnw[l], dbnb[l] = D().bn_bwd_rows(d[:, sl], pre[:, sl], bnw[l].detach(), bnb[l].detach(), stats[2 * l],
-                                               stats[2 * l + 1], True, True, True, dpre[:, sl], ctx.hsb)
+            if not fused:
+                dbnw[l], dbnb[l] = D().bn_bwd_rows(d[:, sl], pre[:, sl], bnw[l].detach(), bnb[l].detach(), stats[2 * l],
+                                                   stats[2 * l + 1], True, True, True, dpre[:, sl], ctx.hsb)
             bs, ld = bsld[l]
             if need[1 + l]:
                 w_t = _conv3x3_dgrad_rows(convw[l], cdt)
diff --git a/include/dclip.h b/include/dclip.h
--- a/include/dclip.h
+++ b/include/dclip.h
@@ -47,7 +47,8 @@
 #define DCLIP_OPT_ATTN_DQ_REDUCE 18
 #define DCLIP_OPT_ATTN_PREP_ORDER 19
 #define DCLIP_OPT_ATTN_BWD_WGS 20
-#define DCLIP_OPT_COUNT 21
+#define DCLIP_OPT_BN_LEVELS 21
+#define DCLIP_OPT_COUNT 22
 int dclip_set_option(int id, int value);
 
 int dclip_layernorm_fwd(const void* x, int x_dt, const float* w, const float* b,
@@ -269,6 +270,14 @@
 int dclip_bn_bwd(int dt, const void* dy, const void* x, int64_t rows, int C, int64_t ld, const float* w,
                  const float* b, const float* mean, const float* rstd, float* ws, void* dx, float* dw,
                  float* db, int relu, const float* gscale, void* stream);
+int64_t dclip_bn_levels_workspace(int64_t rows, int L, int C);
+int dclip_bn_fwd_levels(int dt, const void* x, int64_t rows, int L, int C, int64_t ld, const float* const* w,
+                        const float* const* b, float eps, float momentum, float* const* running_mean,
+                        float* const* running_var, long long* const* num_batches_tracked, float* ws, float* mean,
+                        float* rstd, void* y, int relu, void* stream);
+int dclip_bn_bwd_levels(int dt, const void* dy, const void* x, int64_t rows, int L, int C, int64_t ld,
+                        const float* const* w, const float* const* b, const float* mean, const float* rstd, float* ws,
+                        void* dx, float* dw, float* db, int relu, const float* gscale, void* stream);
 
 #define DCLIP_ADAMW_DESC_WORDS 12
 #define DCLIP_ADAMW_CHUNK 256
```
